# lucidrains/transfusion-pytorch

Hardware: AMD Instinct MI355X
Metric: train samples/sec, dim512 d8 seq1024 text+latent (higher is better)
Workload: dtype bf16; 1 GPU; BASELINE config 2: Transfusion dim=512 depth=8 heads=8 dim_head=64 num_text_tokens=256 dim_latent=384; per-GPU batch 64 x seq 1024 (32 x [24 text tokens + (4,384) latent] per sample); step = pack + fwd + bwd + clip(0.5) + Adam(3e-4) (one GPU: no gradient exchange); global_batch=64, seq_len=1024, parallelism=dp1

## Files before the change

include/tfx.h:

```cpp
#ifndef TFX_H
#define TFX_H
#include <stdint.h>
#ifdef __cplusplus
extern "C" {
#endif

#ifndef TFX_BF16_DEFINED
typedef uint16_t tfx_bf16;
#endif

enum { TFX_EPI_BF16 = 0, TFX_EPI_F32 = 1, TFX_EPI_SILU = 2, TFX_EPI_RESID = 3, TFX_EPI_GEGLU = 4, TFX_EPI_GEGLU_BWD = 5, TFX_EPI_QKV_NORM_ROPE = 6 };

typedef struct {
  const tfx_bf16* A; int32_t lda;
  const tfx_bf16* A2; int32_t lda2; int32_t K1;
  const tfx_bf16* B; int32_t ldb;
  int32_t M, N, K;
  int32_t epi;
  void* C; int32_t ldc;
  void* C2; int32_t ldc2;
  const float* bias;
  const tfx_bf16* R; int32_t ldr; int32_t resid_mapped;
  const int32_t* rowmap;
  const int32_t* a_rowmap;
  const tfx_bf16* aux; int32_t ldaux;
  int32_t qk_heads;
  const float* qk_gamma_q; const float* qk_gamma_k;
  const int32_t* qk_rot_pos; const float* qk_cos; const float* qk_sin;
  float qk_q_scale, qk_norm_scale;
  float* qk_plan; float qk_softcap;
  tfx_bf16* qk_cache; int32_t qk_ld_cache; const int32_t* qk_cache_pos;
  const void* prefetch; int64_t prefetch_bytes;
} tfx_gemm_nt_args;
int tfx_gemm_nt(const tfx_gemm_nt_args* a, void* stream);
int tfx_gemm_nt_plan(const tfx_gemm_nt_args* a, int32_t* kind, int32_t* grid);

int tfx_mfma_peak_probe(const void* ops, float* out, int32_t iters, int32_t blocks, void* stream);

typedef struct {
  const tfx_bf16* A; int32_t lda; int32_t a_cols;
  const tfx_bf16* B; int32_t ldb; int32_t b_cols;
  int32_t M, N, K;
  float* C; int32_t ldc;
  const int32_t* rowmap;
  int32_t k_valid;
  int32_t splits;
  int32_t accumulate;
  float alpha;
  const int32_t* a_rowmap;
  const int32_t* b_rowmap;
  float* colsum;
  int32_t k_group;
  const void* group_next;
} tfx_gemm_tn_args;
int tfx_gemm_tn(const tfx_gemm_tn_args* a, void* stream);
int tfx_gemm_tn_plan(const tfx_gemm_tn_args* a, int32_t* kind, int32_t* tiles, int32_t* splits, int32_t* grid);

typedef struct {
  const tfx_bf16 *q, *k, *v; int32_t ld_q, ld_k, ld_v;
  const tfx_bf16* gate; int32_t ld_gate;
  const int32_t* kv_end;
  const int32_t* q_start;
  tfx_bf16* out; int32_t ld_out;
  float* lse;
  int32_t b, h, n;
  float softcap;
  int32_t n_kv;
  const tfx_bf16* dout; int32_t ld_dout;
  tfx_bf16* do_eff; int32_t ld_do;
  float* delta;
  tfx_bf16* dgate; int32_t ld_dgate;
  tfx_bf16 *dq, *dk, *dv; int32_t ld_dq, ld_dk, ld_dv;
  int32_t order;
  const float* sc_plan;
  const int32_t* q_row0; const int32_t* q_cnt;
  const tfx_bf16* nr_qkv; int32_t nr_ld_qkv;
  tfx_bf16* nr_dqkv; int32_t nr_ld_dqkv;
  const float* nr_gamma_q; const float* nr_gamma_k;
  const int32_t* nr_rot_pos; const float* nr_cos; const float* nr_sin;
  float nr_q_scale, nr_norm_scale;
  float* nr_dgamma_q; float* nr_dgamma_k;
  int32_t laser;
} tfx_attn_args;
int tfx_attn_fwd(const tfx_attn_args* a, void* stream);
int tfx_attn_bwd(const tfx_attn_args* a, void* stream);

int tfx_decode_attn(const tfx_attn_args* a, void* stream);

typedef struct {
  int32_t T, H;
  const tfx_bf16* v; int32_t ld_v;
  tfx_bf16* vl; int32_t ld_vl;
  const int32_t* rowmap;
  float c;
  const tfx_bf16* dvl; int32_t ld_dvl;
  tfx_bf16* dv; int32_t ld_dv;
} tfx_laser_v_args;
int tfx_laser_v_fwd(const tfx_laser_v_args* a, void* stream);
int tfx_laser_v_bwd(const tfx_laser_v_args* a, void* stream);

typedef struct {
  int32_t T, d;
  const tfx_bf16* x; tfx_bf16* u;
  const int32_t* tok_inst;
  const float* table; int32_t ld_table;
  const float* gamma_text;
  float* mean; float* rstd;
  const tfx_bf16* du; tfx_bf16* dx;
  float* dtable;
  float* dgamma_text;
  const int32_t* seg_start; const int32_t* seg_len; int32_t n_seg;
  const tfx_bf16* dx_add;
} tfx_adaln_pre_args;
int tfx_adaln_pre_fwd(const tfx_adaln_pre_args* a, void* stream);
int tfx_adaln_pre_bwd(const tfx_adaln_pre_args* a, void* stream);

typedef struct {
  int32_t T, d;
  const tfx_bf16* x; const tfx_bf16* y; tfx_bf16* out;
  const int32_t* tok_inst;
  const float* table; int32_t ld_table;
  const float* layerscale;
  const tfx_bf16* g; tfx_bf16* dy;
  float* dtable; float* dlayerscale;
  const int32_t* seg_start; const int32_t* seg_len; int32_t n_seg;
  float* dbias;
} tfx_adaln_post_args;
int tfx_adaln_post_fwd(const tfx_adaln_post_args* a, void* stream);
int tfx_adaln_post_bwd(const tfx_adaln_post_args* a, void* stream);

typedef struct {
  int32_t T, H;
  const tfx_bf16* qkv; int32_t ld_qkv;
  tfx_bf16* qk; int32_t ld_qk;
  const float* gamma_q; const float* gamma_k;
  const int32_t* rot_pos;
// ... 54 lines not shown
typedef struct {
  int32_t T, d;
  const tfx_bf16* x; tfx_bf16* y; const float* gamma;
  const tfx_bf16* dy; tfx_bf16* dx; float* dgamma;
} tfx_rmsnorm_args;
int tfx_rmsnorm_fwd(const tfx_rmsnorm_args* a, void* stream);
int tfx_rmsnorm_bwd(const tfx_rmsnorm_args* a, void* stream);

typedef struct {
  int32_t T, d;
  const int32_t* text_ids; const int32_t* tok_inst;
  const tfx_bf16* table;
  tfx_bf16* x;
  const tfx_bf16* dx; float* dtable;
} tfx_embed_args;
int tfx_embed_fwd(const tfx_embed_args* a, void* stream);
int tfx_embed_bwd(const tfx_embed_args* a, void* stream);

typedef struct {
  int32_t R, dl;
  const float* x; const float* eps;
  const int32_t* row_inst; const float* inst_time;
  tfx_bf16* xt; int32_t ld_xt;
  float* flow;
} tfx_noise_mix_args;
int tfx_noise_mix(const tfx_noise_mix_args* a, void* stream);

typedef struct { int32_t I, half; const float* times; const float* w; tfx_bf16* out; int32_t ld; } tfx_fourier_args;
int tfx_fourier(const tfx_fourier_args* a, void* stream);

typedef struct {
  int32_t T, V; const float* logits; int32_t ld;
  const int32_t* labels;
  float grad_scale;
  tfx_bf16* dlogits; int32_t ld_d;
  float* acc;
} tfx_ce_args;
int tfx_ce_fwd_bwd(const tfx_ce_args* a, void* stream);

typedef struct {
  int32_t R, dl; const float* pred; int32_t ld_pred; const float* flow;
  float grad_scale;
  tfx_bf16* dpred; int32_t ld_d;
  float* acc;
  int32_t accumulate;
  const int32_t* row_inst; const float* inst_time; float clean_eps;
  const float* recon_w; const int32_t* recon_inst; const float* recon_time; int32_t recon_mode;
} tfx_mse_args;
int tfx_mse_fwd_bwd(const tfx_mse_args* a, void* stream);
typedef struct {
  int32_t T, d; const tfx_bf16* pred; int32_t ld_pred; const tfx_bf16* target; int32_t ld_target;
  int32_t n_pad, n_valid;
  float grad_scale;
  tfx_bf16* dpred; int32_t ld_d;
  float* acc;
} tfx_cosine_args;
int tfx_cosine_fwd_bwd(const tfx_cosine_args* a, void* stream);
int tfx_output_to_flow(float* pred, const float* x, const float* eps, const int32_t* row_inst, const float* inst_time,
                       int32_t R, int32_t dl, float clean_eps, void* stream);

int tfx_sample_tokens(const float* logits, int32_t ld, int32_t B, int32_t V, float temperature, float min_p, const float* uniforms,
                      const int32_t* active, int32_t* out_ids, void* stream);
int tfx_sample_tokens_range(const float* logits, int32_t ld, int32_t B, int32_t V, int32_t V_draw, float temperature, float min_p, const float* uniforms,
                            const int32_t* active, int32_t* out_ids, void* stream);
int tfx_ode_axpy(const float* y, const float* f_cond, const float* f_uncond, float cfg_scale, float a, float* out, int64_t n, void* stream);
int tfx_ode_stage(const float* y, const float* ym, const float* ctl, int32_t B, int32_t Lc, int32_t dmax, float* x, int32_t H, int32_t Lq, int32_t dl,
                  const int32_t* rows0, void* stream);
int tfx_ode_update(float* y, float* ym, const float* ctl, int32_t B, int32_t Lc, int32_t dmax, const float* pred, int32_t H, int32_t Lq, int32_t dl,
                   float cfg_scale, const float* sel, const int32_t* rows0, void* stream);

typedef struct { const float* src; int32_t ld_src, Rs, Cs; const int32_t* rowmap; tfx_bf16* dst; int32_t ld_dst, Rd, Cd; } tfx_cast_args;
int tfx_cast_rows(const tfx_cast_args* a, void* stream);
int tfx_cast_rows_t(const tfx_cast_args* a, void* stream);
typedef struct { const float* src; int32_t ld_src, Rs, Cs; const int32_t* rowmap; tfx_bf16* dst; int32_t ld_dst, Rd, Cd; int32_t transposed, first_block; } tfx_cast_job;
int tfx_cast_batch(const tfx_cast_job* jobs_dev, int32_t n_jobs, int32_t n_blocks, void* stream);
int tfx_gather_f32(const float* src, const int32_t* map, float* dst, int32_t n, void* stream);
int tfx_onehot_bf16(const int32_t* ids, const int32_t* tok_inst, tfx_bf16* out, int32_t T, int32_t ld, void* stream);
int tfx_scatter_rows_bf16(const tfx_bf16* src, int32_t ld_src, int32_t cols, tfx_bf16* dst, int32_t ld_dst, const int32_t* rowmap, int32_t R, void* stream);
int tfx_f32_to_bf16(const float* src, tfx_bf16* dst, int64_t n, void* stream);
int tfx_cast_block_bf16(const float* src, int32_t ld_src, tfx_bf16* dst, int32_t ld_dst, int32_t R, int32_t C, void* stream);
int tfx_silu_bwd(const tfx_bf16* dy, const tfx_bf16* pre, tfx_bf16* dx, int64_t n, void* stream);
int tfx_colsum_bf16(const tfx_bf16* src, int32_t ld, int32_t R, int32_t C, const int32_t* colmap, const int32_t* rowmap, float* out, void* stream);
int tfx_colsum_f32(const float* src, int32_t ld, int32_t R, int32_t C, float* out, void* stream);
int tfx_add_bf16(const tfx_bf16* a, const tfx_bf16* b, tfx_bf16* out, int64_t n, void* stream);
int tfx_scale_bf16_dev(tfx_bf16* x, int64_t n, const float* scale, void* stream);
int tfx_scale_bf16_copy(const tfx_bf16* src, tfx_bf16* dst, int64_t n, float scale, void* stream);

int tfx_sumsq(const float* g, int64_t n, float* sumsq, void* stream);
typedef struct {
  float* p; const float* g; float* m; float* v; int64_t n;
  float lr, beta1, beta2, eps, weight_decay, max_norm, grad_scale;
  int32_t step; const float* sumsq;
  const int64_t* skip; int32_t nskip;
} tfx_adam_args;
int tfx_adam_step(const tfx_adam_args* a, void* stream);

enum { TFX_SUMSQ_DET_PARTIALS = 1024 };
int tfx_sumsq_det(const float* g, int64_t n, float* partials, float* sumsq, void* stream);
int tfx_muon_plan(int32_t rows, int32_t cols, int32_t* flip, int32_t* m, int32_t* n, int32_t* m_pad, int32_t* n_pad, int32_t* gram_tiles,
                  int32_t* update_tiles, int32_t* prep_blocks);
int tfx_muon_step_launches(int32_t ns_steps, int32_t nmat);
typedef struct {
  int64_t off;
  int64_t s_off, t_off;
  int32_t rows, cols, ld_s, ld_t;
  int32_t blk0;
  float lr_ratio;
} tfx_muon_mat;
typedef struct {
  const tfx_muon_mat* mats; const int32_t* blk_mat; int32_t nmat, nblk;
  const float* g; float* buf; tfx_bf16* ws; float* partials;
  const float* sumsq; float max_norm, grad_scale, momentum; int32_t nesterov;
} tfx_muon_prep_args;
int tfx_muon_prep(const tfx_muon_prep_args* a, void* stream);
int tfx_muon_norm(const tfx_muon_mat* mats, int32_t nmat, const float* partials, float eps, float* inv, void* stream);
typedef struct {
  const tfx_bf16* P; const tfx_bf16* Q; const tfx_bf16* Z; tfx_bf16* C; tfx_bf16* Ct;
  const float* scale_z; const float* scale_acc;
  int32_t M, N, K, ldp, ldq, ldz, ldc, ldct;
  int32_t tile0;
  int32_t reserved;
} tfx_muon_gemm_problem;
int tfx_muon_gemm(const tfx_muon_gemm_problem* table, const int32_t* tile_prob, int32_t ntiles, float alpha, float beta, void* stream);
typedef struct {
  const tfx_muon_mat* mats; const int32_t* blk_mat; int32_t nmat, nblk;
  float* p; const tfx_bf16* ws; float lr, decay;
} tfx_muon_apply_args;
int tfx_muon_apply(const tfx_muon_apply_args* a, void* stream);
int tfx_ema_update(float* ema, const float* online, int64_t n, float decay, void* stream);

int tfx_allreduce_unique_id(void* out128);
int tfx_allreduce_init(int32_t rank, int32_t world, const void* unique_id128);
int tfx_allreduce_run(float* buf, int64_t count, void* stream);
int tfx_allreduce_destroy(void);

typedef struct { const void *p0, *p1, *p2, *p3, *p4; int64_t i0, i1, i2, i3; float f0; int32_t reserved; } tfx_raw_args;
enum { TFX_OP_GEMM_NT = 0, TFX_OP_GEMM_TN = 1, TFX_OP_ATTN_FWD = 2, TFX_OP_ATTN_BWD = 3, TFX_OP_ADALN_PRE_FWD = 4, TFX_OP_ADALN_PRE_BWD = 5,
       TFX_OP_ADALN_POST_FWD = 6, TFX_OP_ADALN_POST_BWD = 7, TFX_OP_QK_NORM_ROPE_FWD = 8, TFX_OP_QK_NORM_ROPE_BWD = 9, TFX_OP_ATTNRES_FWD = 10,
       TFX_OP_ATTNRES_BWD = 11, TFX_OP_RMSNORM_FWD = 12, TFX_OP_RMSNORM_BWD = 13, TFX_OP_EMBED_FWD = 14, TFX_OP_EMBED_BWD = 15,
       TFX_OP_NOISE_MIX = 16, TFX_OP_FOURIER = 17, TFX_OP_CE_FWD_BWD = 18, TFX_OP_MSE_FWD_BWD = 19, TFX_OP_CAST_ROWS = 20, TFX_OP_CAST_ROWS_T = 21,
       TFX_OP_ADAM_STEP = 22, TFX_OP_DECODE_ATTN = 23, TFX_OP_LASER_V_FWD = 24, TFX_OP_LASER_V_BWD = 25, TFX_OP_COSINE_FWD_BWD = 26,
       TFX_OP_OUTPUT_TO_FLOW = 32, TFX_OP_GATHER_F32 = 33, TFX_OP_ONEHOT_BF16 = 34, TFX_OP_SCATTER_ROWS_BF16 = 35, TFX_OP_F32_TO_BF16 = 36,
       TFX_OP_SILU_BWD = 37, TFX_OP_COLSUM_BF16 = 38, TFX_OP_COLSUM_F32 = 39, TFX_OP_ADD_BF16 = 40, TFX_OP_SCALE_BF16_DEV = 41, TFX_OP_CAST_BLOCK_BF16 = 42, TFX_OP_SCALE_BF16_COPY = 43, TFX_OP_ADALN_POST_PRE_FWD = 44, TFX_OP_LAYER_END_FWD = 45,
       TFX_OP_ATTNRES_PREP = 46, TFX_OP_ATTNRES_PULL_BWD = 47, TFX_OP_ATTNRES_FINISH = 52, TFX_OP_ADALN_PRE_POST_BWD = 53,
       TFX_OP_FORK = 48, TFX_OP_JOIN = 49, TFX_OP_JOIN_RECORD = 50, TFX_OP_JOIN_WAIT = 51 };
typedef struct { int32_t op; int32_t stream; const void* args; } tfx_launch;
int tfx_run_list(const tfx_launch* list, int32_t n, void* stream, int32_t* failed_at);
int tfx_graph_create(const tfx_launch* list, int32_t n, void** graph_out);
int tfx_graph_create_single(const tfx_launch* list, int32_t n, void** graph_out);
int tfx_graph_launch(void* graph, void* stream);
int tfx_graph_destroy(void* graph);
int tfx_list_fingerprint(const tfx_launch* list, int32_t n, int64_t* out);
int tfx_set_single_stream(int32_t on);

const char* tfx_version(void);

#ifdef __cplusplus
}
#endif
#endif
```

transfusion_pytorch_amd/capi.py:

```python
from __future__ import annotations

import ctypes
import os
import re

HERE = os.path.dirname(os.path.abspath(__file__))
HEADER = os.path.join(os.path.dirname(HERE), 'include', 'tfx.h')
LIB_PATH = os.environ.get('TFX_LIB') or os.path.join(HERE, 'lib', 'libtfx_hip.so')

_SCALARS = {'int32_t': ctypes.c_int32, 'int64_t': ctypes.c_int64, 'float': ctypes.c_float, 'int': ctypes.c_int}


def _strip_comments(src: str) -> str:
    src = re.sub(r'/\*.*?\*/', '', src, flags=re.S)
    return re.sub(r'//[^\n]*', '', src)


def parse_header(path: str = HEADER):
    src = _strip_comments(open(path).read())
    structs, funcs, enums = {}, {}, {}
    for body in re.findall(r'enum\s*\{(.*?)\}', src, flags=re.S):
        for item in body.split(','):
            if '=' in item:
                k, v = item.split('=')
                enums[k.strip()] = int(v.strip())
    for body, name in re.findall(r'typedef\s+struct\s*\{(.*?)\}\s*(\w+)\s*;', src, flags=re.S):
        fields = []
        for decl in body.split(';'):
            decl = decl.strip()
            if not decl:
                continue
            decl = decl.replace('const ', '')
            m = re.match(r'(\w+)\s*(.*)', decl, flags=re.S)
            base, rest = m.group(1), m.group(2)
            for d in rest.split(','):
                d = d.strip()
                is_ptr = d.startswith('*')
                fname = d.lstrip('* ').strip()
                if is_ptr:
                    fields.append((fname, ctypes.c_void_p))
                else:
                    fields.append((fname, _SCALARS[base]))
        structs[name] = fields
    for ret, name, args in re.findall(r'\b(int|const char\s*\*)\s+(tfx_\w+)\s*\(([^)]*)\)\s*;', src):
        argt = []
        for a in args.split(','):
            a = a.strip().replace('const ', '')
            if a in ('void', ''):
                continue
            if '*' in a:
                argt.append(ctypes.c_void_p)
            else:
                argt.append(_SCALARS[a.split()[0]])
        funcs[name] = (ctypes.c_char_p if 'char' in ret else ctypes.c_int, argt)
    return structs, funcs, enums


STRUCT_FIELDS, FUNCTIONS, ENUMS = parse_header()


def _make_struct(name, fields):
    return type(name, (ctypes.Structure,), {'_fields_': fields})


STRUCTS = {n: _make_struct(n, f) for n, f in STRUCT_FIELDS.items()}
_lib = None


class TfxError(RuntimeError):
    pass


def lib():
    global _lib
    if _lib is None:
        if not os.path.exists(LIB_PATH):
            raise TfxError(f'{LIB_PATH} is missing: build it with `python -m transfusion_pytorch_amd.build` '
                           '(hipcc --offload-arch=gfx950); the Transfusion hot path has no fallback')
        L = ctypes.CDLL(LIB_PATH)
        for fname, (ret, argt) in FUNCTIONS.items():
            fn = getattr(L, fname)
            fn.restype = ret
            fn.argtypes = argt
        _lib = L
    return _lib


def ptr(t):
    return None if t is None else t.data_ptr()


def make_args(struct_name: str, **kw):
    S = STRUCTS[struct_name]
    a = S()
    names = {f for f, _ in STRUCT_FIELDS[struct_name]}
    for k, v in kw.items():
        if k not in names:
            raise KeyError(f'{struct_name} has no field {k}')
        if hasattr(v, 'data_ptr'):
            v = v.data_ptr()
        setattr(a, k, v)
    return a


def check(rc: int, what: str):
    if rc != 0:
        raise TfxError(f'{what} failed with code {rc}')


def call(fn_name: str, args, stream: int):
    rc = getattr(lib(), fn_name)(ctypes.byref(args), ctypes.c_void_p(stream))
    if rc != 0:
        raise TfxError(f'{fn_name} failed with code {rc}')
```

transfusion_pytorch_amd/csrc/gemm.hip:

```cpp
#include "tfx_common.h"
#include "tfx_kernels.h"
#include <type_traits>
#include <cmath>
#include <cstring>
#include <vector>
#include <algorithm>
#include <mutex>

namespace tfx {

constexpr int BM = 128, BN = 128, BK = 64;

template <int EPI> struct Epilogue;

TFX_DEV void store_bf16x4(bf16* dst, f32x4 v) {
  bf16x4 o; o[0] = f2bf(v[0]); o[1] = f2bf(v[1]); o[2] = f2bf(v[2]); o[3] = f2bf(v[3]);
  *(bf16x4*)dst = o;
}

TFX_DEV f32x4 add_bias(const GemmNT& p, int n, f32x4 v) {
  if (p.bias) { f32x4 b = *(const f32x4*)(p.bias + n); v += b; }
  return v;
}

// ... 251 lines not shown
  for (int j = 0; j < 2; j++)
#pragma unroll
    for (int g = 0; g < 4; g++) bias[j][g] = zero4;
  if (p.bias) {
#pragma unroll
    for (int j = 0; j < 2; j++)
#pragma unroll
      for (int g = 0; g < 4; g++) bias[j][g] = *(const f32x4*)(p.bias + min(n_w + j * 32 + 8 * g + 4 * hi, p.N - 4));
  }
  const bool col_ok = n_w + ch * 8 < p.N;
  const int ncol = min(n_w + ch * 8, p.N - 8);
  bf16* sr = st + 4096;
  bf16x8 pre[4];
  auto load_r = [&](int i) {
#pragma unroll
    for (int q = 0; q < 4; q++) pre[q] = *(const bf16x8*)(p.R + (size_t)mr[i][q] * p.ldr + ncol);
  };
  load_r(0);
#pragma unroll
  for (int i = 0; i < NI; i++) {
#pragma unroll
    for (int q = 0; q < 4; q++) {
      const int row = q * 8 + (l >> 3);
      *(bf16x8*)(sr + row * 64 + ((ch ^ ((row >> 1) & 7)) << 3)) = pre[q];
    }
    if (i + 1 < NI) load_r(i + 1);
    bf16* s = st + (i & 1) * 2048;
#pragma unroll
    for (int j = 0; j < 2; j++)
#pragma unroll
      for (int g = 0; g < 4; g++) {
        const int col = j * 32 + 8 * g + 4 * hi;
        const bf16x4 rv = *(const bf16x4*)(sr + r * 64 + (((col >> 3) ^ ((r >> 1) & 7)) << 3) + (col & 7));
        f32x4 v;
#pragma unroll
        for (int e = 0; e < 4; e++) v[e] = acc[i][j][4 * g + e] + bias[j][g][e] + bf2f(rv[e]);
        stage_put4(s, r, col, v);
      }
    bf16x8 v[4];
#pragma unroll
    for (int q = 0; q < 4; q++) {
      const int row = q * 8 + (l >> 3);
      v[q] = *(const bf16x8*)(s + row * 64 + ((ch ^ ((row >> 1) & 7)) << 3));
    }
#pragma unroll
    for (int q = 0; q < 4; q++)
      if (col_ok && mo[i][q] >= 0) *(bf16x8*)((bf16*)p.C + (size_t)mo[i][q] * p.ldc + n_w + ch * 8) = v[q];
  }
}
TFX_DEV void stage_put4_32(bf16* st, int row, int col, f32x4 v) {
  bf16x4 o; o[0] = f2bf(v[0]); o[1] = f2bf(v[1]); o[2] = f2bf(v[2]); o[3] = f2bf(v[3]);
  *(bf16x4*)(st + row * 32 + (((col >> 3) ^ ((row >> 2) & 3)) << 3) + (col & 7)) = o;
}
constexpr int GTAB_N = 4096;
TFX_DEV float gelu_grid(const float* gtab, float g) {
  const float x = g * 128.f;
  const float xr = __builtin_amdgcn_fmed3f(__builtin_rintf(x), -1024.f, 1023.f);
  const float d = x - xr;
  const f32x4 c = *(const f32x4*)(gtab + 4 * ((int)xr + 1024));
  return fmaf(fmaf(c[2], d, c[1]), d, c[0]);
}
TFX_DEV GegluUVH geglu_uvh_grid(const float* gtab, float a, float g) {
  const float x = g * 128.f;
  const float xr = __builtin_amdgcn_fmed3f(__builtin_rintf(x), -1024.f, 1023.f);
  const float d = x - xr;
  const f32x4 c = *(const f32x4*)(gtab + 4 * ((int)xr + 1024));
  const float t = fmaf(c[2], d, c[1]);
  GegluUVH r; r.u = fmaf(t, d, c[0]);
  r.h = a * r.u;
  r.v = (a * 128.f) * fmaf(c[2], d, t);
  return r;
}
template <int EPI, int NI>
TFX_DEV void staged_epilogue_geglu(const GemmNT& p, f32x16 (&acc)[NI][2], int m_w, int n_w, bf16* st, const float* gtab = nullptr, bool use_tab = false) {
  const int l = threadIdx.x & 63, hi = l >> 5, r = l & 31, ch = l & 7;
  int mo[NI][4], mo2[NI][2];
#pragma unroll
  for (int i = 0; i < NI; i++) {
#pragma unroll
    for (int q = 0; q < 4; q++) { const int m = m_w + i * 32 + q * 8 + (l >> 3); mo[i][q] = m < p.M ? (p.rowmap ? p.rowmap[m] : m) : -1; }
#pragma unroll
    for (int q = 0; q < 2; q++) { const int m = m_w + i * 32 + q * 16 + (l >> 2); mo2[i][q] = (EPI == EPI_GEGLU && m < p.M) ? (p.rowmap ? p.rowmap[m] : m) : -1; }
  }
  auto flush64 = [&](const bf16* s, int i, int n_base, int Nout) {
    bf16x8 v[4];
#pragma unroll
    for (int q = 0; q < 4; q++) {
      const int row = q * 8 + (l >> 3);
      v[q] = *(const bf16x8*)(s + row * 64 + ((ch ^ ((row >> 1) & 7)) << 3));
    }
#pragma unroll
    for (int q = 0; q < 4; q++)
      if (n_base + ch * 8 < Nout && mo[i][q] >= 0) *(bf16x8*)((bf16*)p.C + (size_t)mo[i][q] * p.ldc + n_base + ch * 8) = v[q];
  };
  if constexpr (EPI == EPI_GEGLU) {
    f32x4 ba[4], bg[4];
    const f32x4 zero4 = {0.f, 0.f, 0.f, 0.f};
#pragma unroll
    for (int g = 0; g < 4; g++) { ba[g] = zero4; bg[g] = zero4; }
    if (p.bias) {
#pragma unroll
      for (int g = 0; g < 4; g++) { const int n_a = min(n_w + 8 * g + 4 * hi, p.N - 36); ba[g] = *(const f32x4*)(p.bias + n_a); bg[g] = *(const f32x4*)(p.bias + n_a + 32); }
    }
    const int c4 = l & 3;
#pragma unroll
    for (int i = 0; i < NI; i++) {
      bf16* s = st + (i & 1) * 3072;
#pragma unroll
      for (int g = 0; g < 4; g++) {
        const int nl = 8 * g + 4 * hi;
        f32x4 u, v, h;
        if (use_tab) {
#pragma unroll
          for (int e = 0; e < 4; e++) { const GegluUVH t_ = geglu_uvh_grid(gtab, acc[i][0][4 * g + e] + ba[g][e], acc[i][1][4 * g + e] + bg[g][e]); u[e] = t_.u; v[e] = t_.v; h[e] = t_.h; }
        } else {
#pragma unroll
          for (int e = 0; e < 4; e++) { const GegluUVH t_ = geglu_uvh(acc[i][0][4 * g + e] + ba[g][e], acc[i][1][4 * g + e] + bg[g][e]); u[e] = t_.u; v[e] = t_.v; h[e] = t_.h; }
        }
        stage_put4(s, r, nl, u); stage_put4(s, r, 32 + nl, v); stage_put4_32(s + 2048, r, nl, h);
      }
      flush64(s, i, n_w, p.N);
      bf16x8 hv[2];
#pragma unroll
      for (int q = 0; q < 2; q++) {
        const int row = q * 16 + (l >> 2);
        hv[q] = *(const bf16x8*)(s + 2048 + row * 32 + ((c4 ^ ((row >> 2) & 3)) << 3));
      }
      const int feat = (n_w >> 6) * 32 + c4 * 8;
#pragma unroll
      for (int q = 0; q < 2; q++)
        if (n_w < p.N && mo2[i][q] >= 0) *(bf16x8*)((bf16*)p.C2 + (size_t)mo2[i][q] * p.ldc2 + feat) = hv[q];
    }
  } else {
    bf16* sag = st + 2048;
    const int cbase = min(n_w >> 5, (p.N >> 5) - 2) * 64;
    bf16x8 pre[8];
    auto load_aux = [&](int i) {
#pragma unroll
      for (int k = 0; k < 8; k++) {
        const int q = l + 64 * k, row = q >> 4, cc = q & 15;
        const int m = min(m_w + i * 32 + row, p.M - 1);
        pre[k] = *(const bf16x8*)(p.aux + (size_t)m * p.ldaux + cbase + cc * 8);
      }
    };
    load_aux(0);
#pragma unroll
    for (int i = 0; i < NI; i++) {
#pragma unroll
      for (int k = 0; k < 8; k++) {
        const int q = l + 64 * k, row = q >> 4, cc = q & 15;
        *(bf16x8*)(sag + row * 128 + ((cc ^ (row & 15)) << 3)) = pre[k];
      }
      if (i + 1 < NI) load_aux(i + 1);
#pragma unroll
      for (int j = 0; j < 2; j++) {
#pragma unroll
        for (int g = 0; g < 4; g++) {
          const bf16x4 u4 = *(const bf16x4*)(sag + r * 128 + (((j * 8 + g) ^ (r & 15)) << 3) + 4 * hi);
          const bf16x4 v4 = *(const bf16x4*)(sag + r * 128 + (((j * 8 + 4 + g) ^ (r & 15)) << 3) + 4 * hi);
          f32x4 da, dg;
#pragma unroll
          for (int e = 0; e < 4; e++) {
            const float dh = acc[i][j][4 * g + e];
            da[e] = dh * bf2f(u4[e]);
            dg[e] = dh * bf2f(v4[e]);
          }
          stage_put4(st, r, 8 * g + 4 * hi, da); stage_put4(st, r, 32 + 8 * g + 4 * hi, dg);
        }
        if (n_w + j * 32 < p.N) flush64(st, i, ((n_w >> 5) + j) * 64, 2 * p.N);
      }
    }
  }
}
template <int NI, bool GUARD>
TFX_DEV void staged_epilogue_qknr_(const GemmNT& p, f32x16 (&acc)[NI][2], int m_w, int n_w, bf16* st) {
  const int l = threadIdx.x & 63, hi = l >> 5, r = l & 31, ch = l & 7;
  const int hd = p.qk_heads * 64;
  const int which = n_w >= hd;
  const bool col_ok = n_w + ch * 8 < p.N;
  constexpr int NS = 2 * NI;
  auto row_of = [&](int s, int k) { return m_w + (s >> 1) * 32 + (2 * (s & 1) + k) * 8 + (l >> 3); };
  f32x4 g0 = {0.f, 0.f, 0.f, 0.f}, g1 = g0;
  float rs = 0.f;
  int pos_a[2] = {0, 0}, pos_b[2] = {0, 0};
  f32x4 cs_n[2], sn_n[2];
  auto load_pos = [&](int s, int (&pos)[2]) {
#pragma unroll
    for (int k = 0; k < 2; k++) pos[k] = p.qk_rot_pos[min(row_of(s, k), p.M - 1)];
  };
  const bool to_cache = NI == 1 && p.qk_cache != nullptr && which == 1;
  int cpos[NI == 1 ? NS : 1][2];
  if constexpr (NI == 1) {
#pragma unroll
    for (int s = 0; s < NS; s++)
#pragma unroll
      for (int k = 0; k < 2; k++) { const int m = row_of(s, k); cpos[s][k] = (to_cache && m < p.M) ? p.qk_cache_pos[m] : -1; }
  }
  auto load_cs = [&](const int (&pos)[2], f32x4 (&cs)[2], f32x4 (&sn)[2]) {
#pragma unroll
    for (int k = 0; k < 2; k++) {
      cs[k] = *(const f32x4*)(p.qk_cos + (size_t)pos[k] * 32 + ch * 4);
      sn[k] = *(const f32x4*)(p.qk_sin + (size_t)pos[k] * 32 + ch * 4);
    }
  };
  {
    const float* gm = (which ? p.qk_gamma_k : p.qk_gamma_q) + ch * 8;
    g0 = *(const f32x4*)gm; g1 = *(const f32x4*)(gm + 4);
    rs = (p.qk_norm_scale > 0.f ? p.qk_norm_scale : 8.f);
    load_pos(0, pos_a);
    load_cs(pos_a, cs_n, sn_n);
    load_pos(1, pos_a);
    if (NS > 2) load_pos(2, pos_b);
    asm volatile("" ::: "memory");
  }
  bf16x8 v[4];
#pragma unroll
  for (int s = 0; s < NS; s++) {
    const int i = s >> 1, qh = s & 1;
    f32x4 cs[2] = {cs_n[0], cs_n[1]}, sn[2] = {sn_n[0], sn_n[1]};
    {
      if (s + 1 < NS) load_cs(pos_a, cs_n, sn_n);
      pos_a[0] = pos_b[0]; pos_a[1] = pos_b[1];
      if (s + 3 < NS) load_pos(s + 3, pos_b);
      asm volatile("" ::: "memory");
    }
    if (qh == 0) {
      bf16* sbuf = st + (i & 1) * 2048;
#pragma unroll
      for (int j = 0; j < 2; j++)
#pragma unroll
        for (int g = 0; g < 4; g++) {
          f32x4 a4;
#pragma unroll
          for (int e = 0; e < 4; e++) a4[e] = acc[i][j][4 * g + e];
          stage_put4(sbuf, r, j * 32 + 8 * g + 4 * hi, a4);
        }
#pragma unroll
      for (int q = 0; q < 4; q++) {
        const int row = q * 8 + (l >> 3);
        v[q] = *(const bf16x8*)(sbuf + row * 64 + ((ch ^ ((row >> 1) & 7)) << 3));
      }
#pragma unroll
      for (int q = 0; q < 4; q++) {
        const int m = m_w + i * 32 + q * 8 + (l >> 3);
        if (!GUARD || (col_ok && m < p.M)) *(bf16x8*)((bf16*)p.C + (size_t)m * p.ldc + n_w + ch * 8) = v[q];
      }
    }
    {
#pragma unroll
      for (int k = 0; k < 2; k++) {
        float gm[8];
#pragma unroll
// ... 170 lines not shown
      *(u32x4*)(As + buf * BM * BK + off) = ra[i];
      *(u32x4*)(Bs + buf * BN * BK + off) = rb[i];
    }
  };

  f32x16 acc[2][2];
#pragma unroll
  for (int i = 0; i < 2; i++)
#pragma unroll
    for (int j = 0; j < 2; j++)
#pragma unroll
      for (int r = 0; r < 16; r++) acc[i][j][r] = 0.f;

  gload(0);
  sstore(0);
  __syncthreads();

  const int arow0 = wm * 64 + (l & 31), brow0 = wn * 64 + (l & 31);
  for (int kt = 0; kt < nk; kt++) {
    const int cur = kt & 1;
    if (kt + 1 < nk) gload(kt + 1);
    const bf16* as = As + cur * BM * BK;
    const bf16* bs = Bs + cur * BN * BK;
#pragma unroll
    for (int ks = 0; ks < 4; ks++) {
      bf16x8 af[2], bfr[2];
#pragma unroll
      for (int i = 0; i < 2; i++) {
        int ar = arow0 + i * 32, br = brow0 + i * 32;
        af[i] = *(const bf16x8*)(as + ar * BK + (((ks * 2 + hi) ^ ((ar >> 1) & 7)) << 3));
        bfr[i] = *(const bf16x8*)(bs + br * BK + (((ks * 2 + hi) ^ ((br >> 1) & 7)) << 3));
      }
#pragma unroll
      for (int i = 0; i < 2; i++)
#pragma unroll
        for (int j = 0; j < 2; j++)
          acc[i][j] = __builtin_amdgcn_mfma_f32_32x32x16_bf16(bfr[j], af[i], acc[i][j], 0, 0, 0);
    }
    if (kt + 1 < nk) sstore(cur ^ 1);
    __syncthreads();
  }

#pragma unroll
  for (int i = 0; i < 2; i++) {
    const int m = m0 + wm * 64 + i * 32 + (l & 31);
    if (m >= p.M) continue;
    const int mo = p.rowmap ? p.rowmap[m] : m;
    if (mo < 0) continue;
    if constexpr (EPI == EPI_GEGLU) {
#pragma unroll
      for (int g = 0; g < 4; g++) {
        const int n_a = n0 + wn * 64 + 8 * g + 4 * hi;
        if (n_a >= p.N) continue;
        f32x4 a, gt;
#pragma unroll
        for (int e = 0; e < 4; e++) { a[e] = acc[i][0][4 * g + e]; gt[e] = acc[i][1][4 * g + e]; }
        GegluFwd::apply(p, mo, n_a, a, gt);
      }
    } else {
#pragma unroll
      for (int j = 0; j < 2; j++)
#pragma unroll
        for (int g = 0; g < 4; g++) {
          const int n = n0 + wn * 64 + j * 32 + 8 * g + 4 * hi;
          if (n >= p.N) continue;
          f32x4 v;
#pragma unroll
          for (int e = 0; e < 4; e++) v[e] = acc[i][j][4 * g + e];
          Epilogue<EPI>::apply(p, m, mo, n, v);
        }
    }
  }
}

constexpr int TN_BMK = 64;
constexpr int TN_LD = 136;

TFX_DEV int tn_out_col(const GemmTN& p, int k) {
  if (p.k_group <= 0) return k;
  const int c = k & 63;
  return c < p.k_group ? (k >> 6) * p.k_group + c : -1;
}

struct TnBlock { int tile, mbeg, mend; };
TFX_DEV TnBlock tn_block(const GemmTN& p, int ntile) {
  const int per = gridDim.x >> 3;
  const int g = (int)(blockIdx.x & 7) * per + (int)(blockIdx.x >> 3);
  TnBlock b;
  const int chunk = ((p.M + p.splits - 1) / p.splits + TN_BMK - 1) / TN_BMK * TN_BMK;
  const int split = g / ntile;
  b.tile = g - split * ntile;
  b.mbeg = split < p.splits ? min(split * chunk, p.M) : p.M;
  b.mend = min(p.M, b.mbeg + chunk);
  return b;
}

TFX_DEV TnBlock tn_block_ramp(const GemmTN& p, int ntile, int d) {
  if (d <= 0) return tn_block(p, ntile);
  const int per = gridDim.x >> 3;
  const int g = (int)(blockIdx.x & 7) * per + (int)(blockIdx.x >> 3);
  const int S = p.splits, U = p.M / TN_BMK;
  const int tri = d * S * (S - 1) / 2;
  const int c0 = (U - tri) / S, rem = U - tri - c0 * S;
  TnBlock b;
  const int split = g / ntile;
  b.tile = g - split * ntile;
  if (split >= S) { b.mbeg = b.mend = p.M; return b; }
  const int start = c0 * split + d * split * (split - 1) / 2, len = c0 + d * split + (split == S - 1 ? rem : 0);
  b.mbeg = start * TN_BMK; b.mend = (start + len) * TN_BMK;
  return b;
}

__global__ __launch_bounds__(256, 2) void gemm_tn_kernel(GemmTN p) {
  extern __shared__ __attribute__((aligned(16))) char smem_raw[];
  bf16* As = (bf16*)smem_raw;
  bf16* Bs = As + 2 * TN_BMK * TN_LD;

  const int t = threadIdx.x, l = t & 63, w = t >> 6;
  const int wn = w >> 1, wk = w & 1, hi = l >> 5;
  const int ntn = (p.N + 127) / 128, ntk = (p.K + 127) / 128;
  const int ntile = ntn * ntk;
  const TnBlock blk = tn_block(p, ntile);
  const int bid = blk.tile, mbeg = blk.mbeg, mend = blk.mend;
  const int n0 = (bid / ntk) * 128, k0 = (bid % ntk) * 128;
  if (mbeg >= mend) return;
  const int nsteps = (mend - mbeg + TN_BMK - 1) / TN_BMK;

  int srow[4], sch[4];
#pragma unroll
  for (int i = 0; i < 4; i++) { int c = t + 256 * i; srow[i] = c >> 4; sch[i] = c & 15; }
  u32x4 ra[4], rb[4];
  auto gload = [&](int st) {
    int mrow0 = mbeg + st * TN_BMK;
#pragma unroll
    for (int i = 0; i < 4; i++) {
      int m = mrow0 + srow[i];
      int ca = n0 + sch[i] * 8, cb = k0 + sch[i] * 8;
      u32x4 z = {0, 0, 0, 0};
      const bool ok = m < mend;
      const int ma = (ok && p.a_rowmap) ? p.a_rowmap[m] : m;
      const int mb = (ok && p.b_rowmap) ? p.b_rowmap[m] : m;
      ra[i] = (ok && ca < p.a_cols) ? *(const u32x4*)(p.A + (size_t)ma * p.lda + ca) : z;
      rb[i] = (ok && cb < p.b_cols) ? *(const u32x4*)(p.B + (size_t)mb * p.ldb + cb) : z;
    }
  };
  auto sstore = [&](int buf) {
#pragma unroll
    for (int i = 0; i < 4; i++) {
      int off = srow[i] * TN_LD + sch[i] * 8;
      *(u32x4*)(As + buf * TN_BMK * TN_LD + off) = ra[i];
      *(u32x4*)(Bs + buf * TN_BMK * TN_LD + off) = rb[i];
    }
  };

  f32x16 acc[2][2];
#pragma unroll
  for (int i = 0; i < 2; i++)
#pragma unroll
    for (int j = 0; j < 2; j++)
#pragma unroll
      for (int r = 0; r < 16; r++) acc[i][j][r] = 0.f;

  gload(0);
  sstore(0);
  __syncthreads();
  for (int st = 0; st < nsteps; st++) {
    const int cur = st & 1;
    if (st + 1 < nsteps) gload(st + 1);
    const bf16* as = As + cur * TN_BMK * TN_LD;
    const bf16* bs = Bs + cur * TN_BMK * TN_LD;
#pragma unroll
    for (int ks = 0; ks < 4; ks++) {
      const int r0 = ks * 16 + 8 * hi;
      bf16x8 af[2], bfr[2];
#pragma unroll
      for (int i = 0; i < 2; i++) {
        af[i] = lds_tr8(as, TN_LD, r0, r0 + 4, wn * 64 + i * 32);
        bfr[i] = lds_tr8(bs, TN_LD, r0, r0 + 4, wk * 64 + i * 32);
      }
#pragma unroll
      for (int i = 0; i < 2; i++)
#pragma unroll
        for (int j = 0; j < 2; j++)
          acc[i][j] = __builtin_amdgcn_mfma_f32_32x32x16_bf16(af[i], bfr[j], acc[i][j], 0, 0, 0);
    }
    if (st + 1 < nsteps) sstore(cur ^ 1);
    __syncthreads();
  }

#pragma unroll
  for (int i = 0; i < 2; i++)
#pragma unroll
    for (int r = 0; r < 16; r++) {
      const int n = n0 + wn * 64 + i * 32 + (r & 3) + 8 * (r >> 2) + 4 * hi;
      if (n >= p.N) continue;
      const int no = p.rowmap ? p.rowmap[n] : n;
      if (no < 0) continue;
#pragma unroll
      for (int j = 0; j < 2; j++) {
        const int k = k0 + wk * 64 + j * 32 + (l & 31);
        if (k < p.k_valid) {
          float v = acc[i][j][r] * p.alpha;
          const int ko = tn_out_col(p, k);
          if (ko >= 0) atomicAdd(p.C + (size_t)no * p.ldc + ko, v);
        }
      }
    }
}

typedef __attribute__((address_space(1))) const void gbl_void_t;
TFX_DEV void glds16(const bf16* g, bf16* lds_wave_base) {
  __builtin_amdgcn_global_load_lds((gbl_void_t*)g, (lds_void_t*)lds_wave_base, 16, 0, 0);
}

constexpr int PF_BLOCK_BYTES = 64 * 1024;
TFX_DEV bool prefetch_block(const GemmNT& p, int grid0) {
  if ((int)blockIdx.x < grid0) return false;
  const long long o0 = (long long)((int)blockIdx.x - grid0) * PF_BLOCK_BYTES + (long long)threadIdx.x * 64;
  const char* base = (const char*)p.prefetch;
  uint32_t acc = 0;
#pragma unroll
  for (int k = 0; k < PF_BLOCK_BYTES / (256 * 64); k++) {
    const long long o = o0 + (long long)k * 256 * 64;
    if (o + 4 <= (long long)p.prefetch_bytes) acc ^= *(const uint32_t*)(base + o);
  }
  asm volatile("" ::"v"(acc));
  return true;
}
static int prefetch_blocks(const GemmNT& p) {
  if (!p.prefetch || p.prefetch_bytes <= 0) return 0;
  const long long n = ((long long)p.prefetch_bytes + PF_BLOCK_BYTES - 1) / PF_BLOCK_BYTES;
  return (int)(n < 512 ? n : 512);
}

template <int EPI>
__global__ __launch_bounds__(256, 2) void gemm_nt_glds_kernel(GemmNT p, int grid0) {
  extern __shared__ __attribute__((aligned(16))) char smem_raw[];
  if (prefetch_block(p, grid0)) return;
  bf16* As = (bf16*)smem_raw;
  bf16* Bs = As + 2 * BM * BK;

  const int t = threadIdx.x, l = t & 63, hi = l >> 5;
  const int w = __builtin_amdgcn_readfirstlane(t >> 6);
  const int wm = w >> 1, wn = w & 1;
  const int ntn = (p.N + BN - 1) / BN;
  const int bid = xcd_remap(blockIdx.x, grid0);
  const int m0 = (bid / ntn) * BM, n0 = (bid % ntn) * BN;
  const int nk = p.K / BK;

  const bf16 *ga[4], *ga2[4], *gb[4];
#pragma unroll
  for (int j = 0; j < 4; j++) {
    const int row = w * 32 + j * 8 + (l >> 3);
    const int c = (l & 7) ^ ((row >> 1) & 7);
    int rm = min(m0 + row, p.M - 1);
    if (p.a_rowmap) rm = p.a_rowmap[rm];
    const int rn = min(n0 + row, p.N - 1);
    ga[j] = p.A + (size_t)rm * p.lda + c * 8;
    ga2[j] = p.A2 ? p.A2 + (size_t)rm * p.lda2 + c * 8 : nullptr;
    gb[j] = p.B + (size_t)rn * p.ldb + c * 8;
  }
  auto issue = [&](int kt, int buf) {
    const int k0 = kt * BK;
    const bool second = p.A2 && k0 >= p.K1;
#pragma unroll
    for (int j = 0; j < 4; j++) {
      glds16(second ? ga2[j] + (k0 - p.K1) : ga[j] + k0, As + buf * BM * BK + (w * 32 + j * 8) * BK);
      glds16(gb[j] + k0, Bs + buf * BN * BK + (w * 32 + j * 8) * BK);
    }
  };

  f32x16 acc[2][2];
#pragma unroll
  for (int i = 0; i < 2; i++)
#pragma unroll
    for (int j = 0; j < 2; j++)
#pragma unroll
      for (int r = 0; r < 16; r++) acc[i][j][r] = 0.f;

  issue(0, 0);
  const int arow0 = wm * 64 + (l & 31), brow0 = wn * 64 + (l & 31);
  auto ldfrag = [&](const bf16* base, int r, int ks) { return *(const bf16x8*)(base + r * BK + (((ks * 2 + hi) ^ ((r >> 1) & 7)) << 3)); };
  for (int kt = 0; kt < nk; kt++) {
    const int cur = kt & 1;
    asm volatile("s_waitcnt vmcnt(0)" ::: "memory");
    __builtin_amdgcn_s_barrier();
    if (kt + 1 < nk) issue(kt + 1, cur ^ 1);
// ... 728 lines not shown
    TN_CLK(c2)
#ifdef TFX_TN_TIMING
    ti += c2 - c1;
#endif
    const bf16* sa = S + buf * STAGE;
    const bf16* sb = sa + SA * SUBE;
    bf16x8 af[2][FA], bfr[2][FB];
#pragma unroll
    for (int ks = 0; ks < 2; ks++) {
#pragma unroll
      for (int i = 0; i < FA; i++) {
        const int c = (wn * FA + i) * 32;
        af[ks][i] = lds_tr8_swz(sa + (c >> 7) * SUBE, 16 * ks + 8 * hi, 16 * ks + 8 * hi + 4, c & 127);
      }
#pragma unroll
      for (int j = 0; j < FB; j++) {
        const int c = (wk * FB + j) * 32;
        bfr[ks][j] = lds_tr8_swz(sb + (c >> 7) * SUBE, 16 * ks + 8 * hi, 16 * ks + 8 * hi + 4, c & 127);
      }
    }
#pragma unroll
    for (int ks = 0; ks < 2; ks++)
#pragma unroll
      for (int i = 0; i < FA; i++)
#pragma unroll
        for (int j = 0; j < FB; j++) {
          if (!CHECK || (live_a[i] && live_b[j])) acc[i][j] = __builtin_amdgcn_mfma_f32_32x32x16_bf16(af[ks][i], bfr[ks][j], acc[i][j], 0, 0, 0);
          const int idx = (ks * FA + i) * FB + j;
          if (MORE && (idx & 1) && (idx >> 1) < NPW) {
            glds16_asm(gp[idx >> 1], S + nbuf * STAGE + loff[idx >> 1]);
            gp[idx >> 1] += gstep[idx >> 1];
            __builtin_amdgcn_sched_barrier(0);
          }
        }
    if (do_sum) {
#pragma unroll
      for (int ks = 0; ks < 2; ks++)
#pragma unroll
        for (int i = 0; i < (SUM ? FA : 1); i++) accs[i] = __builtin_amdgcn_mfma_f32_32x32x16_bf16(af[ks][i], ones, accs[i], 0, 0, 0);
    }
    buf = buf + 1 == NST ? 0 : buf + 1;
    nbuf = nbuf + 1 == NST ? 0 : nbuf + 1;
  };
  bool all_live = true;
#pragma unroll
  for (int i = 0; i < FA; i++) all_live = all_live && live_a[i];
#pragma unroll
  for (int j = 0; j < FB; j++) all_live = all_live && live_b[j];
  const int n_main = max(0, nst - (NST - 1));
  using yes = std::true_type; using no = std::false_type;
  if (all_live) {
    for (int st = 0; st < n_main; st++) slab(st, yes{}, no{});
    for (int st = n_main; st < nst; st++) slab(st, no{}, no{});
  } else {
    for (int st = 0; st < n_main; st++) slab(st, yes{}, yes{});
    for (int st = n_main; st < nst; st++) slab(st, no{}, yes{});
  }
  TN_STAMP(2)

  int out_row[FA][16];
#pragma unroll
  for (int i = 0; i < FA; i++)
#pragma unroll
    for (int r = 0; r < 16; r++) {
      const int n = n0 + (wn * FA + i) * 32 + (r & 3) + 8 * (r >> 2) + 4 * hi;
      out_row[i][r] = n >= p.N ? -1 : p.rowmap ? p.rowmap[n] : n;
    }
  int out_col[FB];
#pragma unroll
  for (int j = 0; j < FB; j++) {
    const int k = k0 + (wk * FB + j) * 32 + (l & 31);
    out_col[j] = k < p.k_valid ? tn_out_col(p, k) : -1;
  }
#pragma unroll
  for (int i = 0; i < FA; i++)
#pragma unroll
    for (int r = 0; r < 16; r++) {
      const int no = out_row[i][r];
      if (no < 0) continue;
      if (SUM && do_sum && (l & 31) == 0) atomicAdd(p.colsum + no, accs[SUM ? i : 0][r]);
      float* crow = p.C + (size_t)no * p.ldc;
#pragma unroll
      for (int j = 0; j < FB; j++)
        if (out_col[j] >= 0) atomicAdd(crow + out_col[j], acc[i][j][r] * p.alpha);
    }
  TN_STAMP(3)
#ifdef TFX_TN_TIMING
  asm volatile("s_waitcnt vmcnt(0)" ::: "memory");
  TN_STAMP(4)
  if (t == 0) { unsigned long long e = __builtin_readcyclecounter(); tc += stamps[2] - c2; stamps[5] = tw; stamps[6] = ti; stamps[7] = tc; (void)e; }
#endif
#undef TN_STAMP
#undef TN_CLK
}

#define OWT_OUT                                                                                                                                     \
        "=&a"(acc[0][0]), "=&a"(acc[0][1]), "=&a"(acc[0][2]), "=&a"(acc[0][3]), "=&a"(acc[1][0]), "=&a"(acc[1][1]), "=&a"(acc[1][2]), "=&a"(acc[1][3]),    \
        "=&a"(acc[2][0]), "=&a"(acc[2][1]), "=&a"(acc[2][2]), "=&a"(acc[2][3]), "=&a"(acc[3][0]), "=&a"(acc[3][1]), "=&a"(acc[3][2]), "=&a"(acc[3][3]),    \
        "+v"(raA[0]), "+v"(raA[1]), "+v"(raA[2]), "+v"(raA[3]), "+v"(raB[0]), "+v"(raB[1]), "+v"(raB[2]), "+v"(raB[3]),                                     \
        "+v"(voA), "+v"(voB), "+s"(sM), "+s"(cnt), "=&s"(so), "+s"(delta)
#define OWT_IN "s"(rsA), "s"(rsB), "s"(stA), "s"(stB), "s"(ksA), "s"(ksB)
#define OWT_CLOBBER                                                                                                                                 \
        "memory", "scc",                                                                                                                            \
        "v64", "v65", "v66", "v67", "v68", "v69", "v70", "v71", "v72", "v73", "v74", "v75", "v76", "v77", "v78", "v79",                             \
        "v80", "v81", "v82", "v83", "v84", "v85", "v86", "v87", "v88", "v89", "v90", "v91", "v92", "v93", "v94", "v95",                             \
        "v96", "v97", "v98", "v99", "v100", "v101", "v102", "v103", "v104", "v105", "v106", "v107", "v108", "v109", "v110", "v111",                 \
        "v112", "v113", "v114", "v115", "v116", "v117", "v118", "v119", "v120", "v121", "v122", "v123", "v124", "v125", "v126", "v127",             \
        "v128", "v129", "v130", "v131", "v132", "v133", "v134", "v135", "v136", "v137", "v138", "v139", "v140", "v141", "v142", "v143",             \
        "v144", "v145", "v146", "v147", "v148", "v149", "v150", "v151", "v152", "v153", "v154", "v155", "v156", "v157", "v158", "v159",             \
        "v160", "v161", "v162", "v163", "v164", "v165", "v166", "v167", "v168", "v169", "v170", "v171", "v172", "v173", "v174", "v175",             \
        "v176", "v177", "v178", "v179", "v180", "v181", "v182", "v183", "v184", "v185", "v186", "v187", "v188", "v189", "v190", "v191"
template <bool SUM>
TFX_DEV void tn_ow_body(const GemmTN& p, const TnBlock& blk) {
  extern __shared__ __attribute__((aligned(16))) char smem_raw[];
  bf16* S = (bf16*)smem_raw;
  const int t = threadIdx.x, l = t & 63, hi = l >> 5;
  const int w = __builtin_amdgcn_readfirstlane(t >> 6);
  const int wn = w >> 1, wk = w & 1;
  const int ntk = (p.K + 255) / 256;
  const int mbeg = blk.mbeg, mend = blk.mend;
  const int n0 = (blk.tile / ntk) * 256, k0 = (blk.tile % ntk) * 256;
  if (mend - mbeg < 192) return;
  const uint32_t prow = (uint32_t)((w >> 1) * 32 + (l >> 4));
  const uint32_t pchunk = (uint32_t)((l & 15) ^ (((l >> 4) & 3) << 2));
  uint32_t voA = (((uint32_t)mbeg + prow) * (uint32_t)p.lda + (uint32_t)(n0 + (w & 1) * 128) + pchunk * 8u) * 2u;
  const uint32_t ldb = (uint32_t)p.ldb, bcols = (uint32_t)p.b_cols, kb = (uint32_t)k0;
  uint32_t voB = (((uint32_t)mbeg + prow) * ldb + kb + (uint32_t)((w & 1) * 128) + pchunk * 8u) * 2u;
  const uint64_t baseA = (uint64_t)(uintptr_t)p.A, baseB = (uint64_t)(uintptr_t)p.B;
  u32x4 rsA, rsB;
  rsA[0] = __builtin_amdgcn_readfirstlane((uint32_t)baseA); rsA[1] = __builtin_amdgcn_readfirstlane((uint32_t)(baseA >> 32) & 0xffffu);
  rsA[2] = __builtin_amdgcn_readfirstlane(((uint32_t)(p.M - 1) * (uint32_t)p.lda + (uint32_t)p.a_cols) * 2u); rsA[3] = 0x00020000u;
  rsB[0] = __builtin_amdgcn_readfirstlane((uint32_t)baseB); rsB[1] = __builtin_amdgcn_readfirstlane((uint32_t)(baseB >> 32) & 0xffffu);
  rsB[2] = __builtin_amdgcn_readfirstlane(((uint32_t)(p.M - 1) * ldb + bcols) * 2u); rsB[3] = 0x00020000u;
  const uint32_t stA = __builtin_amdgcn_readfirstlane(8u * (uint32_t)p.lda), stB = __builtin_amdgcn_readfirstlane(8u * ldb);
  const uint32_t ksA = __builtin_amdgcn_readfirstlane(128u * (uint32_t)p.lda), ksB = __builtin_amdgcn_readfirstlane(128u * ldb);
  const uint32_t lds0 = (uint32_t)(size_t)(lds_void_t*)S;
  uint32_t sM = __builtin_amdgcn_readfirstlane(lds0 + (uint32_t)((w & 1) * 16384 + (w >> 1) * 8192));
  uint32_t cnt = __builtin_amdgcn_readfirstlane((uint32_t)((mend - mbeg) / 64)), so, delta = 65536u;
  uint32_t raA[4], raB[4];
  {
    const int g = l >> 4, q = l & 15;
    const int row = 8 * (g >> 1) + (q >> 2);
#pragma unroll
    for (int i = 0; i < 4; i++) {
      const int ch = (4 * i + 2 * (g & 1) + ((q & 3) >> 1)) ^ ((row & 3) << 2);
      const uint32_t off = (uint32_t)(row * 256 + ch * 16 + (q & 1) * 8);
      raA[i] = lds0 + (uint32_t)(wn * 16384) + off;
      raB[i] = lds0 + 32768u + (uint32_t)(wk * 16384) + off;
    }
  }
  f32x16 acc[4][4];
  f32x16 accs[2];
  const bool do_sum = SUM && p.colsum != nullptr && k0 == 0;
  if (do_sum) {
    u32x4 ones = {0x3f803f80u, 0x3f803f80u, 0x3f803f80u, 0x3f803f80u};
    if (wk == 0) {
      asm volatile(
#include "gemm_tn_ow_sum01.inc"
          : OWT_OUT, "=&v"(accs[0]), "=&v"(accs[1])
          : OWT_IN, "v"(ones)
          : OWT_CLOBBER);
    } else {
      asm volatile(
#include "gemm_tn_ow_sum23.inc"
          : OWT_OUT, "=&v"(accs[0]), "=&v"(accs[1])
          : OWT_IN, "v"(ones)
          : OWT_CLOBBER);
    }
  } else {
    asm volatile(
#include "gemm_tn_ow_loop.inc"
        : OWT_OUT
        : OWT_IN
        : OWT_CLOBBER);
  }

  int out_col[4];
#pragma unroll
  for (int j = 0; j < 4; j++) {
    const int k = k0 + (wk * 4 + j) * 32 + (l & 31);
    out_col[j] = k < p.k_valid ? tn_out_col(p, k) : -1;
  }
#pragma unroll
  for (int i = 0; i < 4; i++) {
    int out_row[16];
#pragma unroll
    for (int r = 0; r < 16; r++) {
      const int n = n0 + (wn * 4 + i) * 32 + (r & 3) + 8 * (r >> 2) + 4 * hi;
      out_row[r] = n >= p.N ? -1 : p.rowmap ? p.rowmap[n] : n;
    }
#pragma unroll
    for (int r = 0; r < 16; r++) {
      const int no = out_row[r];
      if (no < 0) continue;
      if (SUM && do_sum && (i >> 1) == wk && (l & 31) == 0) atomicAdd(p.colsum + no, accs[i & 1][r]);
      float* crow = p.C + (size_t)no * p.ldc;
#pragma unroll
      for (int j = 0; j < 4; j++)
        if (out_col[j] >= 0) atomicAdd(crow + out_col[j], acc[i][j][r] * p.alpha);
    }
  }
}
template <bool SUM>
__global__ __launch_bounds__(256, 1) void gemm_tn_ow_kernel(GemmTN p, int ramp) {
  const int ntn = (p.N + 255) / 256, ntk = (p.K + 255) / 256;
  tn_ow_body<SUM>(p, tn_block_ramp(p, ntn * ntk, ramp));
}
constexpr int TN_GROUP_MAX = 6;
struct TnGroup { int count; int tile_end[TN_GROUP_MAX]; GemmTN p[TN_GROUP_MAX]; };
template <bool SUM>
__global__ __launch_bounds__(256, 1) void gemm_tn_ow_group_kernel(TnGroup g, int ramp) {
  TnBlock blk = tn_block_ramp(g.p[0], g.tile_end[g.count - 1], ramp);
  int pid = 0, first = 0;
#pragma unroll
  for (int i = 0; i < TN_GROUP_MAX - 1; i++)
    if (i + 1 < g.count && blk.tile >= g.tile_end[i]) { pid = i + 1; first = g.tile_end[i]; }
  blk.tile -= first;
  tn_ow_body<SUM>(g.p[__builtin_amdgcn_readfirstlane(pid)], blk);
}
#undef OWT_OUT
#undef OWT_IN
#undef OWT_CLOBBER

static int tn_auto_splits(int M, int tiles, int kind) {
  constexpr double fill2 = 0.9, fill0 = 0.5;
  const int slots = kind == 2 ? 256 : 512;
  const double want = (kind == 2 ? fill2 : fill0) * slots;
  int s = 1;
  while (tiles * s < want && tiles * (s + 1) <= slots && s < 64 && M / (s + 1) >= 256) s++;
  return s;
}

static bool use_glds() {
  static int v = -1;
  if (v < 0) { const char* e = getenv("TFX_GEMM_GLDS"); v = (e && e[0] == '0') ? 0 : 1; }
  return v == 1;
}

enum { NT_FALLBACK = 0, NT_GLDS = 1, NT_MID = 2, NT_PP = 3, NT_SKINNY = 4, NT_DECODE = 5, NT_OW = 6, NT_OWP = 7 };

static const float* gelu_table() {
  static const float* tab[16] = {nullptr};
  static bool tried[16] = {false};
  static std::mutex mu;
  static int enabled = -1;
  std::lock_guard<std::mutex> lock(mu);
  if (enabled < 0) { const char* e = getenv("TFX_GELU_TABLE"); enabled = e ? atoi(e) : 1; }
  if (!(enabled & 1)) return nullptr;
  int dev = 0;
  if (hipGetDevice(&dev) != hipSuccess || dev < 0 || dev >= 16) return nullptr;
  if (!tried[dev]) {
    tried[dev] = true;
    std::vector<float> h(2 * GTAB_N);
    auto Phi = [](double g) { return 0.5 * erfc(-g * 0.70710678118654752440); };
    auto phi = [](double g) { return 0.39894228040143267794 * exp(-0.5 * g * g); };
    const double st = 1.0 / 128.0;
    for (int i = 0; i < 2048; i++) {
      const double g = (i - 1024) * st;
      h[4 * i] = (float)(g * Phi(g));
// ... 60 lines not shown
  if (!cus[dev]) { hipDeviceProp_t pr; cus[dev] = hipGetDeviceProperties(&pr, dev) == hipSuccess ? pr.multiProcessorCount : 256; }
  const int grid = std::min(cus[dev] / 8 * 8, (tiles + 7) / 8 * 8);
  hipLaunchKernelGGL(gemm_nt_owp_kernel<EPI>, dim3(grid), dim3(256), smem, s, p, PP_STAGGER, tiles);
}
template <int EPI> static void launch_ow(const GemmNT& p, int grid, hipStream_t s) {
  static uint32_t attr_ow = 0;
  const float* gtab = EPI == EPI_GEGLU ? gelu_table() : nullptr;
  const int smem = 2 * (BM2 * BK + BN2 * BK) * 2 + (gtab ? GTAB_N * 8 : 0);
  ensure_smem_attr((const void*)gemm_nt_ow_kernel<EPI>, 2 * (BM2 * BK + BN2 * BK) * 2 + GTAB_N * 8, attr_ow);
  hipLaunchKernelGGL(gemm_nt_ow_kernel<EPI>, dim3(grid), dim3(256), smem, s, p, PP_STAGGER, gtab);
}
template <int EPI> static int launch_nt(const GemmNT& p, hipStream_t s) {
  const NtPlan pl = nt_plan(p);
  const int smem = 2 * (BM * BK + BN * BK) * 2;
  switch (pl.kind) {
    case NT_DECODE: {
      static uint32_t attr_sd = 0;
      const int smem_sd = 4 * SD_ST * SD_SLOT * 2;
      ensure_smem_attr((const void*)gemm_nt_decode_kernel<EPI>, smem_sd, attr_sd);
      hipLaunchKernelGGL(gemm_nt_decode_kernel<EPI>, dim3(pl.grid + prefetch_blocks(p)), dim3(256), smem_sd, s, p, pl.grid);
      break;
    }
    case NT_SKINNY: {
      static uint32_t attr_sk = 0;
      const int smem_sk = SK_ST * SK_STAGE * 2;
      ensure_smem_attr((const void*)gemm_nt_skinny_kernel<EPI>, smem_sk, attr_sk);
      hipLaunchKernelGGL(gemm_nt_skinny_kernel<EPI>, dim3(pl.grid + prefetch_blocks(p)), dim3(256), smem_sk, s, p, pl.grid);
      break;
    }
    case NT_PP: launch_pp<EPI>(p, pl.grid, s); break;
    case NT_OW: if constexpr (EPI == EPI_BF16 || EPI == EPI_F32) launch_ow<EPI>(p, pl.grid, s); break;
    case NT_OWP: if constexpr (EPI == EPI_BF16) launch_owp<EPI>(p, pl.grid, s); break;
    case NT_MID: {
      static uint32_t attr_md = 0;
      const int smem_md = MD_ST * MD_STAGE * 2;
      ensure_smem_attr((const void*)gemm_nt_mid_kernel<EPI>, smem_md, attr_md);
      hipLaunchKernelGGL(gemm_nt_mid_kernel<EPI>, dim3(pl.grid + prefetch_blocks(p)), dim3(256), smem_md, s, p, pl.grid);
      break;
    }
    case NT_GLDS: hipLaunchKernelGGL(gemm_nt_glds_kernel<EPI>, dim3(pl.grid + prefetch_blocks(p)), dim3(256), smem, s, p, pl.grid); break;
    default: hipLaunchKernelGGL(gemm_nt_kernel<EPI>, dim3(pl.grid), dim3(256), smem, s, p); break;
  }
  return (int)hipGetLastError();
}

int gemm_nt_plan(const GemmNT& p, int* kind, int* grid) {
  if (p.K % BK != 0 || (p.A2 && p.K1 % BK != 0) || p.M <= 0 || p.N <= 0) return -1;
  const NtPlan pl = nt_plan(p);
  if (kind) *kind = pl.kind; if (grid) *grid = pl.grid;
  return 0;
}

static bool qknr_fusable(const GemmNT& p) {
  const int kind = nt_plan(p).kind;
  if (kind != NT_PP && kind != NT_DECODE) return false;
  if (kind == NT_PP && p.qk_cache) return false;
  const int hd = p.qk_heads * 64;
  if (p.qk_cache && (!p.qk_cache_pos || (p.qk_ld_cache & 7) || (((uintptr_t)p.qk_cache) & 15) || p.N < 3 * hd)) return false;
  return !p.rowmap && !p.a_rowmap && !p.bias && ((p.ldc | p.ldc2 | p.N) & 7) == 0 && (((uintptr_t)p.C | (uintptr_t)p.C2) & 15) == 0 && 2 * hd <= p.N && p.ldc2 >= 2 * hd;
}
static int gemm_nt_qknr(const GemmNT& p, hipStream_t s) {
  if (p.qk_heads <= 0 || !p.C2 || !p.qk_gamma_q || !p.qk_gamma_k || !p.qk_rot_pos || !p.qk_cos || !p.qk_sin) return -5;
  if (qknr_fusable(p)) {
    const NtPlan pl = nt_plan(p);
    if (pl.kind == NT_PP) { launch_pp<EPI_QKNR>(p, pl.grid, s); return (int)hipGetLastError(); }
    static uint32_t attr_sd = 0;
    const int smem_sd = 4 * SD_ST * SD_SLOT * 2;
    ensure_smem_attr((const void*)gemm_nt_decode_kernel<EPI_QKNR>, smem_sd, attr_sd);
    hipLaunchKernelGGL(gemm_nt_decode_kernel<EPI_QKNR>, dim3(pl.grid + prefetch_blocks(p)), dim3(256), smem_sd, s, p, pl.grid);
    return (int)hipGetLastError();
  }
  GemmNT q = p; q.epi = EPI_BF16; q.C2 = nullptr;
  const int rc = launch_nt<EPI_BF16>(q, s);
  if (rc) return rc;
  tfx_qk_norm_rope_args a;
  memset(&a, 0, sizeof(a));
  a.T = p.M; a.H = p.qk_heads; a.qkv = (const tfx_bf16*)p.C; a.ld_qkv = p.ldc; a.qk = (tfx_bf16*)p.C2; a.ld_qk = p.ldc2;
  a.gamma_q = p.qk_gamma_q; a.gamma_k = p.qk_gamma_k; a.rot_pos = p.qk_rot_pos; a.cos_tab = p.qk_cos; a.sin_tab = p.qk_sin;
  a.q_scale = p.qk_q_scale; a.norm_scale = p.qk_norm_scale; a.sc_plan = p.qk_plan; a.softcap = p.qk_softcap;
  a.cache = p.qk_cache; a.ld_cache = p.qk_ld_cache; a.cache_pos = p.qk_cache_pos;
  return tfx_qk_norm_rope_fwd(&a, (void*)s);
}

int gemm_nt(const GemmNT& p, hipStream_t s) {
  if (p.K % BK != 0 || (p.A2 && p.K1 % BK != 0) || p.M <= 0 || p.N <= 0) return -1;
  if ((p.lda | p.ldb) & 7) return -2;
  switch (p.epi) {
    case EPI_BF16: return launch_nt<EPI_BF16>(p, s);
    case EPI_F32: return launch_nt<EPI_F32>(p, s);
    case EPI_SILU: return launch_nt<EPI_SILU>(p, s);
    case EPI_RESID: return launch_nt<EPI_RESID>(p, s);
    case EPI_GEGLU: return (p.N % 64) ? -3 : launch_nt<EPI_GEGLU>(p, s);
    case EPI_GEGLU_BWD: return (p.N % 64) ? -3 : launch_nt<EPI_GEGLU_BWD>(p, s);
    case EPI_QKNR: return gemm_nt_qknr(p, s);
  }
  return -4;
}

template <bool SUM, int FA, int FB, int WN, int WK, int NST> static void launch_tn_wide(const GemmTN& q, int grid, hipStream_t s) {
  constexpr int smem = NST * (FA * WN + FB * WK) / 4 * MW_ROWS * 128 * 2;
  static uint32_t attr = 0;
  ensure_smem_attr((const void*)gemm_tn_wide_kernel<SUM, FA, FB, WN, WK, NST>, smem, attr);
  hipLaunchKernelGGL((gemm_tn_wide_kernel<SUM, FA, FB, WN, WK, NST>), dim3(grid), dim3(64 * WN * WK), smem, s, q);
}

struct TnPlan { int kind, tiles, splits, grid; };
static int tn_ow_mode();
static bool tn_ow_operands_ok(const GemmTN& q);
static TnPlan tn_plan(const GemmTN& q) {
#ifdef TFX_TN_TIMING
  const bool dma_ok = true;
#else
  const bool dma_ok = use_glds() && q.M % TN_BMK == 0 && !q.a_rowmap && !q.b_rowmap && q.a_cols >= 8 && q.b_cols >= 8;
#endif
  const int t44 = ((q.N + 255) / 256) * ((q.K + 255) / 256), t22 = ((q.N + 127) / 128) * ((q.K + 127) / 128);
  TnPlan pl;
  pl.kind = !dma_ok ? -1 : (t44 >= 8 ? 2 : 0);
  pl.tiles = pl.kind == 2 ? t44 : t22;
  pl.splits = q.splits == 0 ? tn_auto_splits(q.M, pl.tiles, pl.kind) : q.splits;
  pl.grid = (pl.tiles * pl.splits + 7) / 8 * 8;
  if (tn_ow_mode() && pl.kind == 2 && tn_ow_operands_ok(q)) {
    const int chunk = ((q.M + pl.splits - 1) / pl.splits + TN_BMK - 1) / TN_BMK * TN_BMK;
    const int last = q.M % chunk == 0 ? chunk : q.M % chunk;
    if (chunk >= 192 && last >= 192) pl.kind = 3;
  }
  return pl;
}
struct TnGroupPlan { bool ok; int count, tiles, splits, grid; TnGroup g; };
static int tn_ow_mode() {
  static int tnow = -1;
  if (tnow < 0) { const char* e = getenv("TFX_TN_OW"); tnow = e ? atoi(e) : 1; }
  return tnow;
}
static bool tn_ow_operands_ok(const GemmTN& q) {
  const long long lim = 1ll << 32;
  const bool b_ok = q.b_cols >= q.K;
  return use_glds() && q.M % 64 == 0 && !q.a_rowmap && !q.b_rowmap && (((uintptr_t)q.A | (uintptr_t)q.B) & 15) == 0 && ((q.lda | q.ldb | q.a_cols | q.b_cols) & 7) == 0 &&
         (long long)(q.M + 64) * q.lda * 2 < lim && (long long)(q.M + 64) * q.ldb * 2 < lim && q.a_cols >= q.N && b_ok && q.N > 0 && q.K > 0;
}
static TnGroupPlan tn_group_plan(const GemmTN& head) {
  TnGroupPlan gp; memset(&gp, 0, sizeof(gp));
  static int grp = -1;
  if (grp < 0) { const char* e = getenv("TFX_TN_GROUP"); grp = e ? atoi(e) : 1; }
  const GemmTN* q = &head;
  int n = 0, tiles = 0;
  bool ok = grp != 0 && tn_ow_mode() != 0;
  while (q && n < TN_GROUP_MAX) {
    ok = ok && q->M == head.M && tn_ow_operands_ok(*q);
    tiles += ((q->N + 255) / 256) * ((q->K + 255) / 256);
    gp.g.p[n] = *q; gp.g.p[n].group_next = nullptr; gp.g.tile_end[n] = tiles;
    n++;
    q = (const GemmTN*)q->group_next;
  }
  ok = ok && q == nullptr && n >= 2;
  gp.count = n; gp.tiles = tiles; gp.g.count = n;
  if (!ok) return gp;
  gp.splits = head.splits == 0 ? tn_auto_splits(head.M, tiles, 2) : head.splits;
  const int chunk = ((head.M + gp.splits - 1) / gp.splits + TN_BMK - 1) / TN_BMK * TN_BMK;
  const int last = head.M % chunk == 0 ? chunk : head.M % chunk;
  if (chunk < 192 || last < 192) return gp;
  gp.grid = (tiles * gp.splits + 7) / 8 * 8;
  if (head.splits == 0 && tiles * gp.splits < 0.8 * 256) return gp;
  for (int i = 0; i < n; i++) gp.g.p[i].splits = gp.splits;
  gp.ok = true;
  return gp;
}
static int tn_ramp(int M, int tiles, int splits) {
  constexpr int ramp_min = 8;
  int ramp = 0;
  if (splits >= ramp_min && M % TN_BMK == 0) {
    const int S = splits, U = M / TN_BMK;
    ramp = (int)(0.148 * tiles + 0.5);
    while (ramp > 0 && (U - ramp * S * (S - 1) / 2) / S < 8) ramp--;
  }
  return ramp;
}

int gemm_tn_plan(const GemmTN& p, int* kind, int* tiles, int* splits, int* grid) {
  if (p.M <= 0 || p.N <= 0 || p.K <= 0 || p.splits < 0) return -1;
  if (p.group_next) {
    const TnGroupPlan gp = tn_group_plan(p);
    if (gp.ok) { if (kind) *kind = 3; if (tiles) *tiles = gp.tiles; if (splits) *splits = gp.splits; if (grid) *grid = gp.grid; return 0; }
  }
  const TnPlan pl = tn_plan(p);
  if (kind) *kind = pl.kind; if (tiles) *tiles = pl.tiles; if (splits) *splits = pl.splits; if (grid) *grid = pl.grid;
  return 0;
}

int gemm_tn(const GemmTN& p, hipStream_t s) {
  if (p.M <= 0 || p.N <= 0 || p.K <= 0 || p.splits < 0) return -1;
  if ((p.lda | p.ldb | p.a_cols | p.b_cols) & 7) return -2;
  if (p.group_next) {
    const TnGroupPlan gp = tn_group_plan(p);
    if (gp.ok) {
      bool sum = false;
      for (int i = 0; i < gp.count; i++) sum = sum || gp.g.p[i].colsum != nullptr;
      const int ramp = tn_ramp(p.M, gp.tiles, gp.splits);
      static uint32_t attr_g0 = 0, attr_g1 = 0;
      if (sum) { ensure_smem_attr((const void*)gemm_tn_ow_group_kernel<true>, 131072, attr_g1); hipLaunchKernelGGL(gemm_tn_ow_group_kernel<true>, dim3(gp.grid), dim3(256), 131072, s, gp.g, ramp); }
      else { ensure_smem_attr((const void*)gemm_tn_ow_group_kernel<false>, 131072, attr_g0); hipLaunchKernelGGL(gemm_tn_ow_group_kernel<false>, dim3(gp.grid), dim3(256), 131072, s, gp.g, ramp); }
      return (int)hipGetLastError();
    }
    int guard = 0;
    for (const GemmTN* q = &p; q; q = (const GemmTN*)q->group_next) {
      if (++guard > 64) return -7;
      GemmTN one = *q; one.group_next = nullptr;
      const int rc = gemm_tn(one, s);
      if (rc) return rc;
    }
    return 0;
  }
  static uint32_t attr_set = 0;
  const int smem = 2 * 2 * TN_BMK * TN_LD * 2;
  ensure_smem_attr((const void*)gemm_tn_kernel, smem, attr_set);
  GemmTN q = p;
  const TnPlan pl = tn_plan(q);
  q.splits = pl.splits;
  const int kind = pl.kind, grid = pl.grid;
  if (kind == 3) {
    static uint32_t attr_tnow = 0;
    const int ramp = tn_ramp(q.M, pl.tiles, q.splits);
    if (q.colsum) {
      static uint32_t attr_tnows = 0;
      ensure_smem_attr((const void*)gemm_tn_ow_kernel<true>, 131072, attr_tnows);
      hipLaunchKernelGGL(gemm_tn_ow_kernel<true>, dim3(grid), dim3(256), 131072, s, q, ramp);
    } else {
      ensure_smem_attr((const void*)gemm_tn_ow_kernel<false>, 131072, attr_tnow);
      hipLaunchKernelGGL(gemm_tn_ow_kernel<false>, dim3(grid), dim3(256), 131072, s, q, ramp);
    }
  } else if (kind == 2) {
    if (q.colsum) launch_tn_wide<true, 2, 4, 4, 2, 4>(q, grid, s);
    else launch_tn_wide<false, 2, 4, 4, 2, 4>(q, grid, s);
  } else if (kind == 0) {
    if (q.colsum) launch_tn_wide<true, 2, 2, 2, 2, 4>(q, grid, s);
    else launch_tn_wide<false, 2, 2, 2, 2, 4>(q, grid, s);
  }
  else {
    hipLaunchKernelGGL(gemm_tn_kernel, dim3(grid), dim3(256), smem, s, q);
    if (q.colsum)
      return tfx_colsum_bf16((const tfx_bf16*)q.A, q.lda, q.M, q.N, q.rowmap, q.a_rowmap, q.colsum, (void*)s);
  }
  return (int)hipGetLastError();
}

}
```

transfusion_pytorch_amd/csrc/runner.hip:

```cpp
#include <atomic>
#include <hip/hip_runtime.h>
#include <cstdlib>
#include <cstdint>
#include "../../include/tfx.h"

namespace {

inline int run_one(const tfx_launch& l, void* s) {
  const void* a = l.args;
  const tfx_raw_args* r = static_cast<const tfx_raw_args*>(a);
  switch (l.op) {
    case TFX_OP_GEMM_NT:          return tfx_gemm_nt(static_cast<const tfx_gemm_nt_args*>(a), s);
    case TFX_OP_GEMM_TN:          return tfx_gemm_tn(static_cast<const tfx_gemm_tn_args*>(a), s);
    case TFX_OP_ATTN_FWD:         return tfx_attn_fwd(static_cast<const tfx_attn_args*>(a), s);
    case TFX_OP_ATTN_BWD:         return tfx_attn_bwd(static_cast<const tfx_attn_args*>(a), s);
    case TFX_OP_ADALN_PRE_FWD:    return tfx_adaln_pre_fwd(static_cast<const tfx_adaln_pre_args*>(a), s);
    case TFX_OP_ADALN_PRE_BWD:    return tfx_adaln_pre_bwd(static_cast<const tfx_adaln_pre_args*>(a), s);
    case TFX_OP_ADALN_POST_FWD:   return tfx_adaln_post_fwd(static_cast<const tfx_adaln_post_args*>(a), s);
    case TFX_OP_ADALN_POST_BWD:   return tfx_adaln_post_bwd(static_cast<const tfx_adaln_post_args*>(a), s);
    case TFX_OP_QK_NORM_ROPE_FWD: return tfx_qk_norm_rope_fwd(static_cast<const tfx_qk_norm_rope_args*>(a), s);
    case TFX_OP_QK_NORM_ROPE_BWD: return tfx_qk_norm_rope_bwd(static_cast<const tfx_qk_norm_rope_args*>(a), s);
    case TFX_OP_ATTNRES_FWD:      return tfx_attnres_fwd(static_cast<const tfx_attnres_args*>(a), s);
    case TFX_OP_ATTNRES_BWD:      return tfx_attnres_bwd(static_cast<const tfx_attnres_args*>(a), s);
    case TFX_OP_RMSNORM_FWD:      return tfx_rmsnorm_fwd(static_cast<const tfx_rmsnorm_args*>(a), s);
    case TFX_OP_RMSNORM_BWD:      return tfx_rmsnorm_bwd(static_cast<const tfx_rmsnorm_args*>(a), s);
    case TFX_OP_EMBED_FWD:        return tfx_embed_fwd(static_cast<const tfx_embed_args*>(a), s);
    case TFX_OP_EMBED_BWD:        return tfx_embed_bwd(static_cast<const tfx_embed_args*>(a), s);
    case TFX_OP_NOISE_MIX:        return tfx_noise_mix(static_cast<const tfx_noise_mix_args*>(a), s);
    case TFX_OP_FOURIER:          return tfx_fourier(static_cast<const tfx_fourier_args*>(a), s);
    case TFX_OP_CE_FWD_BWD:       return tfx_ce_fwd_bwd(static_cast<const tfx_ce_args*>(a), s);
    case TFX_OP_MSE_FWD_BWD:      return tfx_mse_fwd_bwd(static_cast<const tfx_mse_args*>(a), s);
    case TFX_OP_CAST_ROWS:        return tfx_cast_rows(static_cast<const tfx_cast_args*>(a), s);
    case TFX_OP_CAST_ROWS_T:      return tfx_cast_rows_t(static_cast<const tfx_cast_args*>(a), s);
    case TFX_OP_ADAM_STEP:        return tfx_adam_step(static_cast<const tfx_adam_args*>(a), s);
    case TFX_OP_DECODE_ATTN:      return tfx_decode_attn(static_cast<const tfx_attn_args*>(a), s);
    case TFX_OP_LASER_V_FWD:      return tfx_laser_v_fwd(static_cast<const tfx_laser_v_args*>(a), s);
    case TFX_OP_LASER_V_BWD:      return tfx_laser_v_bwd(static_cast<const tfx_laser_v_args*>(a), s);
    case TFX_OP_COSINE_FWD_BWD:   return tfx_cosine_fwd_bwd(static_cast<const tfx_cosine_args*>(a), s);
    case TFX_OP_OUTPUT_TO_FLOW:
      return tfx_output_to_flow((float*)r->p0, (const float*)r->p1, (const float*)r->p2, (const int32_t*)r->p3, (const float*)r->p4,
                                (int32_t)r->i0, (int32_t)r->i1, r->f0, s);
    case TFX_OP_GATHER_F32:
      return tfx_gather_f32((const float*)r->p0, (const int32_t*)r->p1, (float*)r->p2, (int32_t)r->i0, s);
    case TFX_OP_ONEHOT_BF16:
      return tfx_onehot_bf16((const int32_t*)r->p0, (const int32_t*)r->p1, (tfx_bf16*)r->p2, (int32_t)r->i0, (int32_t)r->i1, s);
    case TFX_OP_SCATTER_ROWS_BF16:
      return tfx_scatter_rows_bf16((const tfx_bf16*)r->p0, (int32_t)r->i0, (int32_t)r->i1, (tfx_bf16*)r->p1, (int32_t)r->i2,
                                   (const int32_t*)r->p2, (int32_t)r->i3, s);
    case TFX_OP_F32_TO_BF16:
      return tfx_f32_to_bf16((const float*)r->p0, (tfx_bf16*)r->p1, r->i0, s);
    case TFX_OP_SILU_BWD:
      return tfx_silu_bwd((const tfx_bf16*)r->p0, (const tfx_bf16*)r->p1, (tfx_bf16*)r->p2, r->i0, s);
    case TFX_OP_COLSUM_BF16:
      return tfx_colsum_bf16((const tfx_bf16*)r->p0, (int32_t)r->i0, (int32_t)r->i1, (int32_t)r->i2, (const int32_t*)r->p1,
                             (const int32_t*)r->p2, (float*)r->p3, s);
    case TFX_OP_COLSUM_F32:
      return tfx_colsum_f32((const float*)r->p0, (int32_t)r->i0, (int32_t)r->i1, (int32_t)r->i2, (float*)r->p1, s);
    case TFX_OP_ADD_BF16:
      return tfx_add_bf16((const tfx_bf16*)r->p0, (const tfx_bf16*)r->p1, (tfx_bf16*)r->p2, r->i0, s);
    case TFX_OP_ADALN_POST_PRE_FWD:
      return tfx_adaln_post_pre_fwd((const tfx_adaln_post_args*)r->p0, (const tfx_adaln_pre_args*)r->p1, s);
    case TFX_OP_LAYER_END_FWD:
      return tfx_layer_end_fwd((const tfx_adaln_post_args*)r->p0, (const tfx_attnres_args*)r->p1, (const tfx_adaln_pre_args*)r->p2, s);
    case TFX_OP_ATTNRES_PREP:
      return tfx_attnres_prep((const tfx_attnres_src*)r->p0, (int32_t)r->i0, (int32_t)r->i1, s);
    case TFX_OP_ATTNRES_FINISH:
      return tfx_attnres_finish((const tfx_attnres_src*)r->p0, (int32_t)r->i0, (int32_t)r->i1, s);
    case TFX_OP_ATTNRES_PULL_BWD:
      return tfx_attnres_pull_bwd((const tfx_attnres_pull_args*)r->p0, (const tfx_adaln_post_args*)r->p1, s);
    case TFX_OP_ADALN_PRE_POST_BWD:
      return tfx_adaln_pre_post_bwd((const tfx_adaln_pre_args*)r->p0, (const tfx_adaln_post_args*)r->p1, s);
    case TFX_OP_CAST_BLOCK_BF16:
      return tfx_cast_block_bf16((const float*)r->p0, (int32_t)r->i0, (tfx_bf16*)r->p1, (int32_t)r->i1, (int32_t)r->i2, (int32_t)r->i3, s);
    case TFX_OP_SCALE_BF16_COPY:
      return tfx_scale_bf16_copy((const tfx_bf16*)r->p0, (tfx_bf16*)r->p1, r->i0, r->f0, s);
    case TFX_OP_SCALE_BF16_DEV:
      return tfx_scale_bf16_dev((tfx_bf16*)r->p0, r->i0, (const float*)r->p1, s);
    default: return -100;
  }
}

struct SideStream {
  hipStream_t stream = nullptr;
  hipEvent_t fork_ev[64] = {}, join_ev[64] = {};
  int ensure() {
    if (stream) return 0;
    int lo = 0, hi = 0;
    (void)hipDeviceGetStreamPriorityRange(&lo, &hi);
    if (hipStreamCreateWithPriority(&stream, hipStreamNonBlocking, lo) != hipSuccess) return -110;
    for (int i = 0; i < 64; ++i)
      if (hipEventCreateWithFlags(&fork_ev[i], hipEventDisableTiming) != hipSuccess ||
          hipEventCreateWithFlags(&join_ev[i], hipEventDisableTiming) != hipSuccess) return -111;
    return 0;
  }
};
constexpr int kMaxDevices = 16;
SideStream g_sides[kMaxDevices];
std::atomic<bool> g_single_stream{false};
thread_local int t_force_single = 0;
inline bool single_stream() { return t_force_single > 0 || g_single_stream.load(std::memory_order_relaxed); }
inline SideStream* side_of_current_device() {
  int dev = 0;
  if (hipGetDevice(&dev) != hipSuccess || dev < 0 || dev >= kMaxDevices) return nullptr;
  return &g_sides[dev];
}

}

extern "C" int tfx_run_list(const tfx_launch* list, int32_t n, void* stream, int32_t* failed_at) {
  if (n < 0 || (n > 0 && !list)) return -1;
  hipStream_t main_s = (hipStream_t)stream;
  SideStream* sp = nullptr;
  auto side = [&](int& rc) -> SideStream* {
    if (!sp && !(sp = side_of_current_device())) { rc = -112; return nullptr; }
    rc = sp->ensure();
    return rc == 0 ? sp : nullptr;
  };
  for (int32_t i = 0; i < n; ++i) {
    const tfx_launch& l = list[i];
    int rc = 0;
    if (!l.args) rc = -2;
    else if (l.op >= TFX_OP_FORK && l.op <= TFX_OP_JOIN_WAIT) {
      if (l.stream < 0 || l.stream >= 64) rc = -3;
      else if (single_stream()) rc = 0;
      else if (SideStream* gs = side(rc)) {
        SideStream& g_side = *gs;
        if (l.op == TFX_OP_FORK) {
          rc = (int)hipEventRecord(g_side.fork_ev[l.stream], main_s);
          if (rc == 0) rc = (int)hipStreamWaitEvent(g_side.stream, g_side.fork_ev[l.stream], 0);
        } else {
          if (l.op != TFX_OP_JOIN_WAIT) rc = (int)hipEventRecord(g_side.join_ev[l.stream], g_side.stream);
          if (rc == 0 && l.op != TFX_OP_JOIN_RECORD) rc = (int)hipStreamWaitEvent(main_s, g_side.join_ev[l.stream], 0);
        }
      }
    } else if (l.stream == 1 && !single_stream()) {
      if (SideStream* gs = side(rc)) rc = run_one(l, (void*)gs->stream);
    } else if (l.stream == 1) {
      rc = run_one(l, stream);
    } else if (l.stream == 0) {
      rc = run_one(l, stream);
    } else rc = -3;
    if (rc != 0) { if (failed_at) *failed_at = i; return rc; }
  }
  return 0;
}

namespace {
hipStream_t g_capture_streams[kMaxDevices] = {};
}
extern "C" int tfx_graph_create(const tfx_launch* list, int32_t n, void** graph_out) {
  if (!graph_out || n <= 0 || !list) return -1;
  *graph_out = nullptr;
  int dev = 0;
  if (hipGetDevice(&dev) != hipSuccess || dev < 0 || dev >= kMaxDevices) return -112;
  hipStream_t& g_capture_stream = g_capture_streams[dev];
  if (!g_capture_stream && hipStreamCreateWithFlags(&g_capture_stream, hipStreamNonBlocking) != hipSuccess) return -120;
// ... 97 lines not shown
```

transfusion_pytorch_amd/csrc/tokenwise.hip:

```cpp
#include "tfx_kernels.h"
#include <map>
#include <mutex>
#include <utility>
#include <cstdlib>

namespace tfx {

constexpr int WAVES = 4;
constexpr int MAXB = 1024;

template <int NC> struct Row {
  float v[NC][8];
};

template <int NC> TFX_DEV void load_row(Row<NC>& r, const bf16* p, int d, int lane) {
#pragma unroll
  for (int i = 0; i < NC; i++) {
    int c = lane + 64 * i;
    if (c * 8 < d) {
      bf16x8 x = *(const bf16x8*)(p + c * 8);
#pragma unroll
      for (int e = 0; e < 8; e++) r.v[i][e] = bf2f(x[e]);
    } else {
#pragma unroll
// ... 1762 lines not shown
  if (i >= n) return;
  float x = bf2f(pre[i]), s = sigmoidf_(x);
  dx[i] = f2bf(bf2f(dy[i]) * s * (1.f + x * (1.f - s)));
}
__global__ void add_bf16_k(const bf16* a, const bf16* b, bf16* o, long long n) {
  long long i = ((long long)blockIdx.x * blockDim.x + threadIdx.x) * 8;
  if (i + 7 < n) {
    bf16x8 x = *(const bf16x8*)(a + i), y = *(const bf16x8*)(b + i), r;
#pragma unroll
    for (int e = 0; e < 8; e++) r[e] = f2bf(bf2f(x[e]) + bf2f(y[e]));
    *(bf16x8*)(o + i) = r;
  } else for (; i < n; i++) o[i] = f2bf(bf2f(a[i]) + bf2f(b[i]));
}

__global__ void scale_bf16_dev_k(bf16* x, long long n, const float* scale) {
  const float sc = *scale;
  if (sc == 1.f) return;
  long long i = ((long long)blockIdx.x * blockDim.x + threadIdx.x) * 8;
  if (i + 7 < n) {
    bf16x8 v = *(const bf16x8*)(x + i);
#pragma unroll
    for (int e = 0; e < 8; e++) v[e] = f2bf(bf2f(v[e]) * sc);
    *(bf16x8*)(x + i) = v;
  } else for (; i < n; i++) x[i] = f2bf(bf2f(x[i]) * sc);
}

template <typename T> __global__ __launch_bounds__(256) void colsum_k(const T* src, int ld, int R, int C, const int* colmap, const int* rowmap, float* out, int rows_per_block) {
  __shared__ float s[4][64];
  const int cx = threadIdx.x & 63, ry = threadIdx.x >> 6;
  const int c = blockIdx.x * 64 + cx;
  const int rbeg = blockIdx.y * rows_per_block, rend = min(R, rbeg + rows_per_block);
  float a = 0.f;
  if (c < C) for (int r = rbeg + ry; r < rend; r += 4) a += (float)src[(size_t)(rowmap ? rowmap[r] : r) * ld + c];
  s[ry][cx] = a;
  __syncthreads();
  if (ry == 0 && c < C) {
    float v = s[0][cx] + s[1][cx] + s[2][cx] + s[3][cx];
    int co = colmap ? colmap[c] : c;
    if (co >= 0 && v != 0.f) atomicAdd(out + co, v);
  }
}

__global__ __launch_bounds__(512) void colsum8_k(const bf16* src, int ld, int R, int C, const int* colmap, const int* rowmap, float* out, int rows_per_block) {
  __shared__ float s[8][64][9];
  const int cx = threadIdx.x & 63, ry = threadIdx.x >> 6;
  const int c0 = (blockIdx.x * 64 + cx) * 8;
  const int rbeg = blockIdx.y * rows_per_block, rend = min(R, rbeg + rows_per_block);
  float a[8];
#pragma unroll
  for (int e = 0; e < 8; e++) a[e] = 0.f;
  if (c0 < C) {
    int r = rbeg + ry;
    for (; r + 56 < rend; r += 64) {
      bf16x8 v[8];
#pragma unroll
      for (int u = 0; u < 8; u++) v[u] = *(const bf16x8*)(src + (size_t)(rowmap ? rowmap[r + 8 * u] : r + 8 * u) * ld + c0);
#pragma unroll
      for (int u = 0; u < 8; u++)
#pragma unroll
        for (int e = 0; e < 8; e++) a[e] += bf2f(v[u][e]);
    }
    for (; r < rend; r += 8) {
      bf16x8 v = *(const bf16x8*)(src + (size_t)(rowmap ? rowmap[r] : r) * ld + c0);
#pragma unroll
      for (int e = 0; e < 8; e++) a[e] += bf2f(v[e]);
    }
  }
#pragma unroll
  for (int e = 0; e < 8; e++) s[ry][cx][e] = a[e];
  __syncthreads();
  {
    const int cc = threadIdx.x >> 3, e = threadIdx.x & 7;
    const int col = (blockIdx.x * 64 + cc) * 8 + e;
    if (col < C) {
      float v = 0.f;
#pragma unroll
      for (int y = 0; y < 8; y++) v += s[y][cc][e];
      const int co = colmap ? colmap[col] : col;
      if (co >= 0 && v != 0.f) atomicAdd(out + co, v);
    }
  }
}

__global__ __launch_bounds__(256) void sumsq_k(const float* g, long long n, float* out) {
  __shared__ float sacc[WAVES];
  float s = 0.f;
  for (long long i = ((long long)blockIdx.x * blockDim.x + threadIdx.x) * 4; i < n; i += (long long)gridDim.x * blockDim.x * 4) {
    if (i + 3 < n) { f32x4 v = *(const f32x4*)(g + i); s += v[0] * v[0] + v[1] * v[1] + v[2] * v[2] + v[3] * v[3]; }
    else for (long long j = i; j < n; j++) s += g[j] * g[j];
  }
  s = wave_sum(s);
  if ((threadIdx.x & 63) == 0) sacc[threadIdx.x >> 6] = s;
  __syncthreads();
  if (threadIdx.x == 0) { float a = 0.f; for (int i = 0; i < WAVES; i++) a += sacc[i]; atomicAdd(out, a); }
}

__global__ __launch_bounds__(256) void adam_k(tfx_adam_args p, float step_size, float inv_sqrt_bc2) {
  const long long i = ((long long)blockIdx.x * blockDim.x + threadIdx.x) * 4;
  if (i >= p.n) return;
  if (p.nskip > 0) {
    int lo = 0, hi = p.nskip;
    while (lo < hi) { const int mid = (lo + hi) >> 1; if (p.skip[2 * mid + 1] > i) hi = mid; else lo = mid + 1; }
    if (lo < p.nskip && p.skip[2 * lo] <= i) return;
  }
  float coef = p.grad_scale;
  if (p.max_norm > 0.f) {
    float norm = sqrtf(p.sumsq[0]) * p.grad_scale;
    coef *= fminf(1.f, p.max_norm / (norm + 1e-6f));
  }
  if (i + 4 <= p.n) {
    const f32x4 g4 = *(const f32x4*)(p.g + i), w4 = *(const f32x4*)(p.p + i);
    f32x4 m4 = *(const f32x4*)(p.m + i), v4 = *(const f32x4*)(p.v + i), o4;
#pragma unroll
    for (int e = 0; e < 4; e++) {
      float g = g4[e] * coef;
      if (p.weight_decay != 0.f) g += p.weight_decay * w4[e];
      m4[e] = p.beta1 * m4[e] + (1.f - p.beta1) * g;
      v4[e] = p.beta2 * v4[e] + (1.f - p.beta2) * g * g;
      o4[e] = w4[e] - step_size * m4[e] / (sqrtf(v4[e]) * inv_sqrt_bc2 + p.eps);
    }
    *(f32x4*)(p.m + i) = m4; *(f32x4*)(p.v + i) = v4; *(f32x4*)(p.p + i) = o4;
  } else {
    for (long long j = i; j < p.n; j++) {
      float g = p.g[j] * coef;
      const float w = p.p[j];
      if (p.weight_decay != 0.f) g += p.weight_decay * w;
      const float m = p.beta1 * p.m[j] + (1.f - p.beta1) * g;
      const float v = p.beta2 * p.v[j] + (1.f - p.beta2) * g * g;
      p.m[j] = m; p.v[j] = v;
      p.p[j] = w - step_size * m / (sqrtf(v) * inv_sqrt_bc2 + p.eps);
    }
  }
}

__global__ __launch_bounds__(256) void output_to_flow_k(float* pred, const float* x, const float* eps, const int* row_inst, const float* inst_time,
                                                        int R, int dl, float clean_eps) {
  const int i = blockIdx.x * blockDim.x + threadIdx.x;
  if (i >= R * dl) return;
  const int r = i / dl;
  const float t = inst_time[row_inst[r]];
  const float noised = eps ? x[i] * t + eps[i] * (1.f - t) : x[i];
  pred[i] = (pred[i] - noised) / fmaxf(1.f - t, clean_eps);
}

__global__ __launch_bounds__(256) void ema_k(float* ema, const float* online, long long n, float decay) {
  const long long i = ((long long)blockIdx.x * blockDim.x + threadIdx.x) * 4;
  if (i + 4 <= n) {
    f32x4 e = *(const f32x4*)(ema + i); const f32x4 o = *(const f32x4*)(online + i);
#pragma unroll
    for (int k = 0; k < 4; k++) e[k] = o[k] + decay * (e[k] - o[k]);
    *(f32x4*)(ema + i) = e;
  } else {
    for (long long j = i; j < n; j++) ema[j] = online[j] + decay * (ema[j] - online[j]);
  }
}

TFX_DEV float laser_factor(float x, float c, float ic, float* th_out) {
  const float th = tanhf(x * ic);
  *th_out = th;
  return expf(c * th);
}
__global__ __launch_bounds__(256) void laser_v_fwd_k(tfx_laser_v_args p, unsigned nch) {
  const unsigned gid = blockIdx.x * blockDim.x + threadIdx.x;
  const unsigned cpr = (unsigned)p.H * 8;
  if (gid >= nch) return;
  const unsigned t = gid / cpr, c8 = gid - t * cpr;
// ... 175 lines not shown
int tfx_qk_norm_rope_bwd(const tfx_qk_norm_rope_args* a, void* s) {
  long long nthreads = (long long)a->T * 2 * a->H * 8;
  if (nthreads >= (1ll << 31)) return -3;
  long long g = (nthreads + 1023) / 1024;
  const long long cap = 256;
  if (g > cap) g = cap;
  hipLaunchKernelGGL(qk_norm_rope_bwd_k, dim3((unsigned)g), dim3(1024), 0, ST(s), *a); RET();
}
int tfx_noise_mix(const tfx_noise_mix_args* a, void* s) {
  long long n = (long long)a->R * a->ld_xt; if (n == 0) return 0;
  hipLaunchKernelGGL(noise_mix_k, dim3((unsigned)((n + 255) / 256)), dim3(256), 0, ST(s), *a); RET();
}
int tfx_fourier(const tfx_fourier_args* a, void* s) { if (a->I == 0) return 0; hipLaunchKernelGGL(fourier_k, dim3(a->I), dim3(256), 0, ST(s), *a); RET(); }
int tfx_ce_fwd_bwd(const tfx_ce_args* a, void* s) {
  int g = grid_tokens(a->T); if (g > 1024) g = 1024;
  hipLaunchKernelGGL(ce_k, dim3(g), dim3(256), 0, ST(s), *a); RET();
}
int tfx_mse_fwd_bwd(const tfx_mse_args* a, void* s) {
  long long n = (long long)a->R * a->ld_d; if (n == 0) return 0;
  long long g = (n + 255) / 256; if (g > 2048) g = 2048;
  hipLaunchKernelGGL(mse_k, dim3((unsigned)g), dim3(256), 0, ST(s), *a); RET();
}
int tfx_cosine_fwd_bwd(const tfx_cosine_args* a, void* s) {
  if (!a || a->T < 0 || a->d <= 0 || a->d > 2048 || (a->d % 64) || (a->ld_pred % 8) || (a->ld_target % 8) || (a->ld_d % 8) || a->ld_pred < a->d || a->ld_target < a->d || a->ld_d < a->d) return -1;
  if (!a->pred || !a->target || !a->dpred || !a->acc || a->n_pad < 0 || a->n_valid < 0) return -2;
  if (a->T == 0) return 0;
  DISPATCH_NC(a->d, hipLaunchKernelGGL(cosine_k<NC>, dim3(grid_capped(a->T)), dim3(256), 0, ST(s), *a)); RET();
}
int tfx_cast_rows(const tfx_cast_args* a, void* s) {
  long long n = (long long)a->Rd * a->ld_dst; if (n == 0) return 0;
  hipLaunchKernelGGL(cast_rows_k, dim3((unsigned)((n + 255) / 256)), dim3(256), 0, ST(s), *a); RET();
}
int tfx_cast_rows_t(const tfx_cast_args* a, void* s) {
  hipLaunchKernelGGL(cast_rows_t_k, dim3((a->ld_dst + 31) / 32, (a->Rd + 31) / 32), dim3(256), 0, ST(s), *a); RET();
}
int tfx_cast_batch(const tfx_cast_job* jobs_dev, int32_t n_jobs, int32_t n_blocks, void* s) {
  if (n_jobs <= 0 || n_blocks <= 0) return 0;
  hipLaunchKernelGGL(cast_batch_k, dim3(n_blocks), dim3(256), 0, ST(s), jobs_dev, n_jobs); RET();
}
int tfx_onehot_bf16(const int32_t* ids, const int32_t* tok_inst, tfx_bf16* out, int32_t T, int32_t ld, void* s) {
  if (T == 0) return 0; if (ld % 8) return -1;
  long long n = (long long)T * ld / 8;
  hipLaunchKernelGGL(onehot_k, dim3((unsigned)((n + 255) / 256)), dim3(256), 0, ST(s), ids, tok_inst, out, T, ld); RET();
}
int tfx_scatter_rows_bf16(const tfx_bf16* src, int32_t ld_src, int32_t cols, tfx_bf16* dst, int32_t ld_dst, const int32_t* rowmap, int32_t R, void* s) {
  if (R == 0) return 0; if (cols % 8 || ld_src % 8 || ld_dst % 8) return -1;
  long long n = (long long)R * (cols / 8);
  hipLaunchKernelGGL(scatter_rows_k, dim3((unsigned)((n + 255) / 256)), dim3(256), 0, ST(s), src, ld_src, cols, dst, ld_dst, rowmap, R); RET();
}
int tfx_gather_f32(const float* src, const int32_t* map, float* dst, int32_t n, void* s) {
  if (n == 0) return 0; hipLaunchKernelGGL(gather_f32_k, dim3((n + 255) / 256), dim3(256), 0, ST(s), src, map, dst, n); RET();
}
int tfx_f32_to_bf16(const float* src, tfx_bf16* dst, int64_t n, void* s) {
  if (n == 0) return 0; hipLaunchKernelGGL(f32_to_bf16_k, dim3((unsigned)((n / 4 + 256) / 256)), dim3(256), 0, ST(s), src, dst, (long long)n); RET();
}
int tfx_silu_bwd(const tfx_bf16* dy, const tfx_bf16* pre, tfx_bf16* dx, int64_t n, void* s) {
  if (n == 0) return 0; hipLaunchKernelGGL(silu_bwd_k, dim3((unsigned)((n + 255) / 256)), dim3(256), 0, ST(s), dy, pre, dx, (long long)n); RET();
}
int tfx_add_bf16(const tfx_bf16* a, const tfx_bf16* b, tfx_bf16* o, int64_t n, void* s) {
  if (n == 0) return 0; hipLaunchKernelGGL(add_bf16_k, dim3((unsigned)((n / 8 + 256) / 256)), dim3(256), 0, ST(s), a, b, o, (long long)n); RET();
}
int tfx_scale_bf16_dev(tfx_bf16* x, int64_t n, const float* scale, void* s) {
  if (n == 0) return 0;
  if (!x || !scale) return -1;
  hipLaunchKernelGGL(scale_bf16_dev_k, dim3((unsigned)((n / 8 + 256) / 256)), dim3(256), 0, ST(s), x, (long long)n, scale); RET();
}
static inline int colsum_rows_per_block(int R) { int rpb = (R + 63) / 64; return rpb < 4 ? 4 : rpb; }
int tfx_colsum_bf16(const tfx_bf16* src, int32_t ld, int32_t R, int32_t C, const int32_t* colmap, const int32_t* rowmap, float* out, void* s) {
  if (R == 0 || C == 0) return 0;
  if (C % 8 == 0 && ld % 8 == 0) {
    const int gx = (C + 511) / 512;
    int gy = 768 / gx; if (gy < 1) gy = 1;
    int rpb8 = (R + gy - 1) / gy; if (rpb8 < 64) rpb8 = 64;
    hipLaunchKernelGGL(colsum8_k, dim3(gx, (R + rpb8 - 1) / rpb8), dim3(512), 0, ST(s), src, ld, R, C, colmap, rowmap, out, rpb8); RET();
  }
  int rpb = colsum_rows_per_block(R);
  hipLaunchKernelGGL(colsum_k<bf16>, dim3((C + 63) / 64, (R + rpb - 1) / rpb), dim3(256), 0, ST(s), src, ld, R, C, colmap, rowmap, out, rpb); RET();
}
int tfx_colsum_f32(const float* src, int32_t ld, int32_t R, int32_t C, float* out, void* s) {
  if (R == 0 || C == 0) return 0;
  int rpb = colsum_rows_per_block(R);
  hipLaunchKernelGGL(colsum_k<float>, dim3((C + 63) / 64, (R + rpb - 1) / rpb), dim3(256), 0, ST(s), src, ld, R, C, (const int*)nullptr, (const int*)nullptr, out, rpb); RET();
}
int tfx_sumsq(const float* g, int64_t n, float* out, void* s) {
  if (n == 0) return 0;
  long long blocks = (n / 4 + 255) / 256; if (blocks > 2048) blocks = 2048; if (blocks < 1) blocks = 1;
  hipLaunchKernelGGL(sumsq_k, dim3((unsigned)blocks), dim3(256), 0, ST(s), g, (long long)n, out); RET();
}
int tfx_adam_step(const tfx_adam_args* a, void* s) {
  if (a->n == 0) return 0;
  if (((uintptr_t)a->p | (uintptr_t)a->g | (uintptr_t)a->m | (uintptr_t)a->v) & 15) return -1;
  if (a->nskip < 0 || (a->nskip > 0 && !a->skip)) return -1;
  const double bc1 = 1.0 - pow((double)a->beta1, (double)a->step), bc2 = 1.0 - pow((double)a->beta2, (double)a->step);
  const long long nthr = (a->n + 3) / 4;
  hipLaunchKernelGGL(adam_k, dim3((unsigned)((nthr + 255) / 256)), dim3(256), 0, ST(s), *a, (float)(a->lr / bc1), (float)(1.0 / sqrt(bc2))); RET();
}
int tfx_output_to_flow(float* pred, const float* x, const float* eps, const int32_t* row_inst, const float* inst_time,
                       int32_t R, int32_t dl, float clean_eps, void* s) {
  if (R <= 0 || dl <= 0) return 0;
  if ((long long)R * dl >= (1ll << 31)) return -1;
  hipLaunchKernelGGL(output_to_flow_k, dim3((unsigned)(((long long)R * dl + 255) / 256)), dim3(256), 0, ST(s), pred, x, eps, row_inst, inst_time, R, dl, clean_eps); RET();
}
int tfx_ema_update(float* ema, const float* online, int64_t n, float decay, void* s) {
  if (n <= 0) return 0;
  if (((uintptr_t)ema | (uintptr_t)online) & 15) return -1;
  hipLaunchKernelGGL(ema_k, dim3((unsigned)(((n + 3) / 4 + 255) / 256)), dim3(256), 0, ST(s), ema, online, (long long)n, decay); RET();
}
int tfx_gemm_nt(const tfx_gemm_nt_args* a, void* s) { return gemm_nt(*a, ST(s)); }
int tfx_gemm_tn(const tfx_gemm_tn_args* a, void* s) { return gemm_tn(*a, ST(s)); }
int tfx_gemm_nt_plan(const tfx_gemm_nt_args* a, int32_t* kind, int32_t* grid) { return gemm_nt_plan(*a, kind, grid); }
int tfx_gemm_tn_plan(const tfx_gemm_tn_args* a, int32_t* kind, int32_t* tiles, int32_t* splits, int32_t* grid) { return gemm_tn_plan(*a, kind, tiles, splits, grid); }
int tfx_attn_fwd(const tfx_attn_args* a, void* s) { return attn_fwd(*a, ST(s)); }
int tfx_attn_bwd(const tfx_attn_args* a, void* s) { return attn_bwd(*a, ST(s)); }
int tfx_mfma_peak_probe(const void* ops, float* out, int32_t iters, int32_t blocks, void* s) {
  if (!ops || !out || iters <= 0 || blocks <= 0) return -1;
  hipLaunchKernelGGL(mfma_peak_k, dim3(blocks), dim3(256), 0, ST(s), (const bf16x8*)ops, out, iters); RET();
}
int tfx_laser_v_fwd(const tfx_laser_v_args* a, void* s) {
  if (!a || a->T < 0 || a->H <= 0 || !(a->c > 0.f)) return -1;
  if (a->T == 0) return 0;
  if (!a->v || !a->vl || ((a->ld_v | a->ld_vl) & 7) || a->ld_v < a->H * 64 || a->ld_vl < a->H * 64 || (((uintptr_t)a->v | (uintptr_t)a->vl) & 15)) return -2;
  const long long nch = (long long)a->T * a->H * 8;
  if (nch >= (1ll << 31)) return -4;
  hipLaunchKernelGGL(laser_v_fwd_k, dim3((unsigned)((nch + 255) / 256)), dim3(256), 0, ST(s), *a, (unsigned)nch); RET();
}
int tfx_laser_v_bwd(const tfx_laser_v_args* a, void* s) {
  if (!a || a->T < 0 || a->H <= 0 || !(a->c > 0.f)) return -1;
  if (a->T == 0) return 0;
  if (!a->v || !a->dvl || !a->dv || ((a->ld_v | a->ld_dvl | a->ld_dv) & 7) || a->ld_v < a->H * 64 || a->ld_dvl < a->H * 64 || a->ld_dv < a->H * 64 ||
      (((uintptr_t)a->v | (uintptr_t)a->dvl | (uintptr_t)a->dv) & 15)) return -2;
  const long long nch = (long long)a->T * a->H * 8;
  if (nch >= (1ll << 31)) return -4;
  hipLaunchKernelGGL(laser_v_bwd_k, dim3((unsigned)((nch + 255) / 256)), dim3(256), 0, ST(s), *a, (unsigned)nch); RET();
}
const char* tfx_version(void) { return "tfx-hip gfx950 r4-laser-muon-selfflow"; }

}
```

transfusion_pytorch_amd/engine.py:

```python
from __future__ import annotations

import ctypes
import os
import weakref

import torch

from . import capi
from .params import ModelDims, ParamStore, pad_to

BF16 = torch.bfloat16
E = capi.ENUMS


def _p(t, *idx):
    for i in idx:
        t = t[i]
    return t.data_ptr()


def skip_sources(md: ModelDims):
    stack, src = [], {}
    for i in range(md.depth):
        layer = i + 1
        if layer <= md.depth // 2:
            stack.append(i)
        elif md.has_skip(i):
            src[i] = stack.pop()
    assert not stack
    return src




_LAUNCH = capi.STRUCTS['tfx_launch']
_RAW = capi.STRUCTS['tfx_raw_args']


def raw_args(fn_name: str, values):
    argt = capi.FUNCTIONS[fn_name][1][:-1]
    assert len(argt) == len(values), f'{fn_name}: {len(values)} arguments for {len(argt)} parameters'
    r = _RAW()
    np_, ni, nf = 0, 0, 0
    for ty, v in zip(argt, values):
        if ty is ctypes.c_void_p:
            setattr(r, f'p{np_}', v); np_ += 1
        elif ty is ctypes.c_float:
            assert nf == 0
            r.f0 = v; nf += 1
        else:
            setattr(r, f'i{ni}', v); ni += 1
    return r


class Side(tuple):
    """a launch that runs on the library's side stream (include/tfx.h `tfx_launch.stream` = 1): the weight-gradient GEMMs, next to
    the data-gradient chain on the caller's stream.  Unpacks like any other (entry point, args) item."""


_AUTO_AFTER = 2
TRAIN_GRAPH = os.environ.get('TFX_TRAIN_GRAPH', '0') == '1'
_SYNC_OPS = {'tfx_fork': 'TFX_OP_FORK', 'tfx_join': 'TFX_OP_JOIN', 'tfx_join_record': 'TFX_OP_JOIN_RECORD', 'tfx_join_wait': 'TFX_OP_JOIN_WAIT'}
_DUMMY = ctypes.c_int32(0)


class LaunchList(list):
    _image = None
    _graphs = None
    meta = None

    def graph(self, lo: int, hi: int):
        if self._graphs is None:
            self._graphs = {}
        g = self._graphs.get((lo, hi))
        if g is None:
            arr = self.native()
            out = ctypes.c_void_p()
            rc = capi.lib().tfx_graph_create(ctypes.byref(arr, lo * ctypes.sizeof(_LAUNCH)), hi - lo, ctypes.byref(out))
            if rc != 0 or not out.value:
                raise capi.TfxError(f'tfx_graph_create failed with code {rc}')
            g = self._graphs[(lo, hi)] = out.value
        return g

    def invalidate_graphs(self):
        for g in (self._graphs or {}).values():
            capi.lib().tfx_graph_destroy(ctypes.c_void_p(g))
        self._graphs = None
        for st in (self._auto or {}).values():
            if st[1]:
                capi.lib().tfx_graph_destroy(ctypes.c_void_p(st[1]))
        self._auto = None

    _auto = None

    def replay_auto(self, lo: int, hi: int, sp) -> bool:
        lib = capi.lib()
        arr = self.native()
        fp = ctypes.c_int64()
        rc = lib.tfx_list_fingerprint(ctypes.byref(arr, lo * ctypes.sizeof(_LAUNCH)), hi - lo, ctypes.byref(fp))
        if rc != 0:
            return False
        if self._auto is None:
            self._auto = {}
        st = self._auto.get((lo, hi))
        if st is None or st[0] != fp.value:
            if st is not None and st[1]:
                lib.tfx_graph_destroy(ctypes.c_void_p(st[1]))
            self._auto[(lo, hi)] = [fp.value, None, 0]
            return False
        st[2] += 1
        if st[1] is None:
            if st[2] < _AUTO_AFTER:
                return False
            out = ctypes.c_void_p()
            rc = lib.tfx_graph_create_single(ctypes.byref(arr, lo * ctypes.sizeof(_LAUNCH)), hi - lo, ctypes.byref(out))
# ... 530 lines not shown
                    self._nt(C, algo_k=dl, A=lt['ndpred'], lda=dlp, B=S[f'outp_t{t}'], ldb=dlp, M=r, N=d, K=dlp, epi=E['TFX_EPI_BF16'], C=lt['dpx'], ldc=d)
                    self._tn(C, r, d, dl, A=lt['dpx'], lda=d, a_cols=d, B=lt['xt'], ldb=dlp, b_cols=dlp, C=gp(f'latent_to_model_projs.{t}.weight'), ldc=dl)
                    self._raw(C, lib.tfx_colsum_bf16, lt['dpx'].data_ptr(), d, r, d, None, None, gp(f'latent_to_model_projs.{t}.bias'))
        self._nt(L, algo_k=md.vocab, A=self.dlogits, lda=md.vp, B=S['logits_t'], ldb=md.vp, M=T, N=d, K=md.vp, epi=E['TFX_EPI_BF16'], C=self.dembed, ldc=d)
        self._tn(L, T, md.vocab, d, A=self.dlogits, lda=md.vp, a_cols=md.vp, B=self.embed, ldb=d, b_cols=d, C=gp('to_text_logits.weight'), ldc=d)
        for t, r in self.R.items():
            dl = md.dim_latents[t]; dlp = pad_to(dl, 64); lt = self.lat[t]
            if t in self.ext:
                self._nt(L, A=lt['gemb'], lda=d, B=S['eye'], ldb=d, M=r, N=d, K=d, epi=E['TFX_EPI_RESID'], C=self.dembed, ldc=d,
                         R=self.dembed, ldr=d, resid_mapped=1, rowmap=self.row_tok[t])
                continue
            self._nt(L, algo_k=dl, A=lt['dpred'], lda=dlp, B=S[f'outp_t{t}'], ldb=dlp, M=r, N=d, K=dlp, epi=E['TFX_EPI_RESID'], C=self.dembed, ldc=d,
                     R=self.dembed, ldr=d, resid_mapped=1, rowmap=self.row_tok[t])
            self._tn(L, r, dl, d, A=lt['dpred'], lda=dlp, a_cols=dlp, B=self.embed, ldb=d, b_cols=d, b_rowmap=self.row_gat[t],
                     C=gp(f'model_to_latent_projs.{t}.weight'), ldc=d)
        self.tap_final = len(L)
        self._k(L, 'tfx_rmsnorm_bwd', 'tfx_rmsnorm_args', T=T, d=d, x=self.xres[D], gamma=pp('transformer.norm.gamma'), dy=self.dembed,
                dx=self.gfin, dgamma=gp('transformer.norm.gamma'))
        self._hbm(L, 3)
        src = skip_sources(md)
        pushed = set(src.values())
        g = self.gfin
        side = self.side
        def sync(op, slot):
            if side:
                L.append((op, slot))
        pull = self.pull
        if pull:
            self.dsum = torch.empty(D, T, device=ps.device, dtype=torch.float32)
            self.wtab = torch.empty(2, D, d, device=ps.device, dtype=torch.float32)
            self.nbytes += self.dsum.numel() * 4 + self.wtab.numel() * 4
            SRC = capi.STRUCTS['tfx_attnres_src']
            recs = (SRC * D)()
            for j in range(D):
                pj = f'transformer.layers.{j}.3'
                gj = self.gfin if j == D - 1 else (self.gx[j + 1] if md.has_skip(j + 1) else self.dH[j + 2])
                for k, v in dict(g=gj, save=self.arsave[j], dsum=self.dsum[j], w=self.wtab[0, j], dw=self.wtab[1, j], gamma=pp(f'{pj}.norm_keys.gamma'),
                                 pq=pp(f'{pj}.pseudo_queries'), dgamma=gp(f'{pj}.norm_keys.gamma'), dpq=gp(f'{pj}.pseudo_queries'), L=j + 2).items():
                    setattr(recs[j], k, v.data_ptr() if hasattr(v, 'data_ptr') else v)
            raw = torch.frombuffer(bytearray(ctypes.string_at(ctypes.addressof(recs), ctypes.sizeof(recs))), dtype=torch.uint8)
            self._src_tab = raw.to(ps.device)
            self._src_size = ctypes.sizeof(SRC)
            self._raw(L, lib.tfx_attnres_prep, self._src_tab.data_ptr(), D, d)
        self._pull_args = {}
        def pull_launch(l, out_own, add, dh, post):
            j0 = max(l - 1, 0)
            ns = D - j0
            export = ns > 8 or d > 512
            if export and not hasattr(self, 'k1buf'):
                self.k1buf = torch.zeros(T, 32, device=ps.device, dtype=BF16); self.nbytes += self.k1buf.numel() * 2
            a = capi.make_args('tfx_attnres_pull_args', T=T, d=d, l=l, n_src=ns, h=self.hid[l], src=self._src_tab.data_ptr() + j0 * self._src_size,
                               out_own=out_own, out_err=self.arerr[l - 1] if out_own is not None else None, add=add, dh=dh,
                               seg_start=self.seg_start, seg_len=self.seg_len, n_seg=0, k1=self.k1buf if export else None, ld_k1=32)
            self._seg_args.append(a)
            self._pull_args[l] = a
            self._keep = getattr(self, '_keep', []) + [a, post]
            self._raw(L, lib.tfx_attnres_pull_bwd, ctypes.addressof(a), ctypes.addressof(post) if post is not None else None)
            self._hbm(L, ns + 6 if post is not None else ns + 4, 12 * ns * T)
            if export:
                self._tn(L, T, ns, d, A=self.k1buf, lda=32, a_cols=32, B=self.hid[l], ldb=d, b_cols=d, C=self.wtab[1, j0], ldc=d)
        for i in range(D - 1, -1, -1):
            p = f'transformer.layers.{i}'
            x_in = self.xres[i]
            x_a = self.xa[i] if md.has_skip(i) else x_in
            (ta, dta), (tf, dtf) = self._tab(i, 0), self._tab(i, 1)
            par = i % len(self.dag_p)
            dy_f, dy_a, dag, dqkvg = self.dy_f[par], self.dy_a[par], self.dag_p[par], self.dqkvg_p[par]
            if i + 2 <= D - 1:
                sync('tfx_join_wait', i + 2)
            G = self.dH[i + 1]
            a_postf = capi.make_args('tfx_adaln_post_args', T=T, d=d, y=self.yf[i], tok_inst=self.tok_inst, table=tf, ld_table=nt3,
                                     layerscale=pp(f'{p}.2.layerscale'), g=G, dy=dy_f, dtable=dtf, dlayerscale=gp(f'{p}.2.layerscale'),
                                     seg_start=self.seg_start, seg_len=self.seg_len, n_seg=0, dbias=gp(f'{p}.2.fn.net.3.bias'))
            self._seg_args.append(a_postf)
            if pull:
                pull_launch(i + 1, self.xres[i + 1], None, G, a_postf)
            else:
                g2 = self.dskip[i + 1] if (i + 1) in pushed else None
                self._k(L, 'tfx_attnres_bwd', 'tfx_attnres_args', T=T, d=d, L=i + 2, hiddens=self.hid, stride_h=T * d,
                        gamma=pp(f'{p}.3.norm_keys.gamma'), pq=pp(f'{p}.3.pseudo_queries'), g=g, g2=capi.ptr(g2), dhiddens=self.dH, stride_dh=T * d,
                        first=1 if i == D - 1 else 0, dgamma=gp(f'{p}.3.norm_keys.gamma'), dpq=gp(f'{p}.3.pseudo_queries'))
                L.append(('tfx_adaln_post_bwd', a_postf))
            self._nt(L, algo_n=di, A=dy_f, lda=d, B=S[f'ff2_t{i}'], ldb=d, M=T, N=dip, K=d, epi=E['TFX_EPI_GEGLU_BWD'], C=dag, ldc=2 * dip,
                     aux=self.ag[i], ldaux=2 * dip)
            sync('tfx_fork', 2 * i)
            ff_grp = [(d, di, dict(A=dy_f, lda=d, a_cols=d, B=self.hm[i], ldb=dip, b_cols=dip, C=gp(f'{p}.2.fn.net.3.weight'), ldc=di)),
                      (2 * dip, d, dict(algo_n=2 * di, A=dag, lda=2 * dip, a_cols=2 * dip, B=self.uf[i], ldb=d, b_cols=d, rowmap=gmap,
                                        C=gp(f'{p}.2.fn.net.0.weight'), ldc=d, colsum=gp(f'{p}.2.fn.net.0.bias')))]
            self._tn_group(L, T, ff_grp, side=side)
            self._nt(L, algo_k=2 * di, A=dag, lda=2 * dip, B=S[f'ff1_t{i}'], ldb=2 * dip, M=T, N=d, K=2 * dip, epi=E['TFX_EPI_BF16'], C=self.du, ldc=d)
            a_pref = capi.make_args('tfx_adaln_pre_args', T=T, d=d, x=self.xb[i], tok_inst=self.tok_inst, table=tf, ld_table=nt3,
                                    gamma_text=pp(f'{p}.2.layernorm_gamma'), mean=_p(self.stats, 2, i), rstd=_p(self.stats, 3, i), du=self.du, dx=G,
                                    dtable=dtf, dgamma_text=gp(f'{p}.2.layernorm_gamma'), seg_start=self.seg_start, seg_len=self.seg_len, n_seg=0)
            a_posta = capi.make_args('tfx_adaln_post_args', T=T, d=d, y=self.ya[i], tok_inst=self.tok_inst, table=ta, ld_table=nt3,
                                     layerscale=pp(f'{p}.1.layerscale'), g=G, dy=dy_a, dtable=dta, dlayerscale=gp(f'{p}.1.layerscale'),
                                     seg_start=self.seg_start, seg_len=self.seg_len, n_seg=0)
            self._seg_args += [a_pref, a_posta]
            self._keep = getattr(self, '_keep', []) + [a_pref, a_posta]
            self._raw(L, lib.tfx_adaln_pre_post_bwd, ctypes.addressof(a_pref), ctypes.addressof(a_posta))
            self._hbm(L, 6)
            self._nt(L, algo_n=md.hd, A=dy_a, lda=d, B=S[f'out_t{i}'], ldb=d, M=T, N=hd, K=d, epi=E['TFX_EPI_BF16'], C=self.dog, ldc=hd)
            gam = (lambda nm: S[f'g{nm}{i}']) if md.dim_head != 64 else (lambda nm: pp(f'{p}.1.fn.{nm}_norm.gamma'))
            if os.environ.get('TFX_ATTN_QKNR', '1') != '0':
                self._k(L, 'tfx_attn_bwd', 'tfx_attn_args', **self._attn_kw(i, bwd=True), nr_qkv=self.qkvg[i], nr_ld_qkv=ldq, nr_dqkv=dqkvg, nr_ld_dqkv=ldq,
                        nr_gamma_q=gam('q'), nr_gamma_k=gam('k'), nr_rot_pos=self.rot_pos, nr_cos=0, nr_sin=0, nr_q_scale=md.dim_head ** -0.5,
                        nr_norm_scale=md.dim_head ** 0.5, nr_dgamma_q=gp(f'{p}.1.fn.q_norm.gamma'), nr_dgamma_k=gp(f'{p}.1.fn.k_norm.gamma'))
                self._rope_attn_args = getattr(self, '_rope_attn_args', []) + [L[-1][1]]
            else:
                self._k(L, 'tfx_attn_bwd', 'tfx_attn_args', **self._attn_kw(i, bwd=True))
                self._k(L, 'tfx_qk_norm_rope_bwd', 'tfx_qk_norm_rope_args', T=T, H=H, qkv=self.qkvg[i], ld_qkv=ldq, gamma_q=gam('q'),
                        gamma_k=gam('k'), rot_pos=self.rot_pos, cos_tab=0, sin_tab=0, q_scale=md.dim_head ** -0.5, norm_scale=md.dim_head ** 0.5,
                        dqk=self.dqk, ld_dqk=2 * hd, dqkv=dqkvg, ld_dqkv=ldq, dgamma_q=gp(f'{p}.1.fn.q_norm.gamma'), dgamma_k=gp(f'{p}.1.fn.k_norm.gamma'))
                self._rope_args = getattr(self, '_rope_args', []) + [L[-1][1]]
                L.meta = L.meta or {}
                L.meta[len(L) - 1] = ('hbm', 3 * 2 * T * hd * 2)
            if md.laser:
                dv = dqkvg.data_ptr() + 2 * 2 * hd
                self._k(L, 'tfx_laser_v_bwd', 'tfx_laser_v_args', T=T, H=H, v=_p(self.qkvg, i) + 2 * 2 * hd, ld_v=ldq, c=md.laser,
                        dvl=dv, ld_dvl=ldq, dv=dv, ld_dv=ldq)
                L.meta = L.meta or {}
                L.meta[len(L) - 1] = ('hbm', 3 * T * hd * 2)
            self._nt(L, algo_k=md.nq, A=dqkvg, lda=ldq, B=S[f'qkvg_t{i}'], ldb=ldq, M=T, N=d, K=ldq, epi=E['TFX_EPI_BF16'], C=self.du, ldc=d)
            self._k(L, 'tfx_adaln_pre_bwd', 'tfx_adaln_pre_args', T=T, d=d, x=x_a, tok_inst=self.tok_inst, table=ta, ld_table=nt3,
                    gamma_text=pp(f'{p}.1.layernorm_gamma'), mean=_p(self.stats, 0, i), rstd=_p(self.stats, 1, i), du=self.du, dx=G,
                    dtable=dta, dgamma_text=gp(f'{p}.1.layernorm_gamma'), seg_start=self.seg_start, seg_len=self.seg_len, n_seg=0,
                    dx_add=self.dskip[i] if (pull and i in pushed) else None)
            self._hbm(L, 4 + (1 if (pull and i in pushed) else 0))
            self._seg_args.append(L[-1][1])
            sync('tfx_fork', 2 * i + 1)
            grp = [(d, hd, dict(A=dy_a, lda=d, a_cols=d, B=self.og[i], ldb=hd, b_cols=hd, C=gp(f'{p}.1.fn.to_out.1.weight'), ldc=md.hd,
                                k_group=0 if md.dim_head == 64 else md.dim_head)),
                   (md.nqk, d, dict(algo_n=md.nq, A=dqkvg, lda=ldq, a_cols=ldq, B=self.ua[i], ldb=d, b_cols=d, C=gp(f'{p}.1.fn.to_qk.0.weight'), ldc=d,
                                    rowmap=ps._maps['heads'] if md.dim_head != 64 else None))]
            if md.has_skip(i):
                sk = self.xres[src[i]]
                grp.append((d, d, dict(A=G, lda=d, a_cols=d, B=x_in, ldb=d, b_cols=d, C=gp(f'{p}.0.weight'), ldc=2 * d)))
                grp.append((d, d, dict(A=G, lda=d, a_cols=d, B=sk, ldb=d, b_cols=d, C=gp(f'{p}.0.weight', d), ldc=2 * d)))
            self._tn_group(L, T, grp, side=side)
            per = -(-D // self.dp_groups) if self.dp_groups > 0 else D
            if I > 0 and i % per == 0:
                hi = min(i + per, D)
                off, cols = i * 2 * 3 * d, (hi - i) * 2 * 3 * d
                w_item = lambda it: L.append(Side(it) if side else it)
                w_item((lib.tfx_cast_block_bf16, (self.dtables.data_ptr() + 4 * off, nt3, self.dtab_bf.data_ptr() + 2 * off, nt3, I, cols)))
                self._tn(L, I, cols, 4 * d, side=side, A=self.dtab_bf.data_ptr() + 2 * off, lda=nt3, a_cols=cols, B=self.cond, ldb=4 * d, b_cols=4 * d,
                         C=gp(f'{p}.1.to_film.weight'), ldc=4 * d)
                w_item((lib.tfx_colsum_f32, (self.dtables.data_ptr() + 4 * off, nt3, I, cols, gp(f'{p}.1.to_film.bias'))))
            sync('tfx_join_record', i)
            if self.dp_groups > 0:
                if i % per == 0:
                    sync('tfx_join_wait', i)
                    self.bwd_cuts.append((len(L), i, min(i + per, D) - 1))
            if md.has_skip(i):
                st = S[f'skip_t{i}']
                self._nt(L, A=G, lda=d, B=st, ldb=d, M=T, N=d, K=d, epi=E['TFX_EPI_RESID'], C=self.gx[i], ldc=d, R=G, ldr=d)
                self._nt(L, A=G, lda=d, B=st[d:], ldb=d, M=T, N=d, K=d, epi=E['TFX_EPI_BF16'], C=self.dskip[src[i]], ldc=d)
                g = self.gx[i]
            else:
                g = G
        sync('tfx_join', 63)
        if pull:
            pull_launch(0, None, g, self.dx0, None)
            self._raw(L, lib.tfx_attnres_finish, self._src_tab.data_ptr(), D, d)
        else:
            self._raw(L, lib.tfx_add_bf16, g.data_ptr(), self.dH[0].data_ptr(), self.dx0.data_ptr(), T * d)
            if 0 in pushed:
                self._raw(L, lib.tfx_add_bf16, self.dx0.data_ptr(), self.dskip[0].data_ptr(), self.dx0.data_ptr(), T * d)
        self._raw(L, lib.tfx_onehot_bf16, self.text_ids.data_ptr(), self.tok_inst.data_ptr(), self.onehot.data_ptr(), T, md.vp)
        self._x0_param_grads(L, self.dx0)
        if I > 0:
            self._nt(L, A=self.dtab_bf, lda=nt3, B=S['ada_t'], ldb=nt3, M=I, N=4 * d, K=nt3, epi=E['TFX_EPI_BF16'], C=self.dcond, ldc=4 * d)
            self._raw(L, lib.tfx_silu_bwd, self.dcond.data_ptr(), self.pre.data_ptr(), self.dpre.data_ptr(), I * 4 * d)
            self._tn(L, I, 4 * d, d + 1, A=self.dpre, lda=4 * d, a_cols=4 * d, B=self.fe, ldb=md.kf, b_cols=md.kf,
                     C=gp('transformer.to_time_cond.1.weight'), ldc=d + 1)
            self._raw(L, lib.tfx_colsum_bf16, self.dpre.data_ptr(), 4 * d, I, 4 * d, None, None, gp('transformer.to_time_cond.1.bias'))

    def _x0_param_grads(self, L, dx0):
        md, T, d = self.md, self.T, self.md.dim
        gp, lib = self.ps.grad_ptr, capi.lib()
        self._tn(L, T, md.vocab, d, A=self.onehot, lda=md.vp, a_cols=md.vp, B=dx0, ldb=d, b_cols=d, C=gp('text_embed.weight'), ldc=d)
        for t, r in self.R.items():
            dl = md.dim_latents[t]; dlp = pad_to(dl, 64); lt = self.lat[t]
            if dl == d or t in self.ext:
                continue
            self._tn(L, r, d, dl, A=dx0, lda=d, a_cols=d, a_rowmap=self.row_gat[t], B=lt['xt'], ldb=dlp, b_cols=dlp,
                     C=gp(f'latent_to_model_projs.{t}.weight'), ldc=dl)
            cs = [dx0.data_ptr(), d, int(self.noise_args[t].R), d, None, self.row_tok[t].data_ptr(), gp(f'latent_to_model_projs.{t}.bias')]
            self._rows_dep[t].append((cs, 2))
            L.append((lib.tfx_colsum_bf16, cs))

    def set_taps(self, grads: dict, n_true: int):
        D, d = self.md.depth, self.md.dim
        self.clear_taps()
        if not grads:
            return
        if not self.pull:
            raise NotImplementedError('hidden taps need the pull-form AttentionResidual backward (depth <= 32 and dim <= 1024): the push form has no '
                                      'place where a hidden\'s gradient is formed once')
        for k, g in grads.items():
            assert 0 <= k <= D + 1
            buf = self.tap_buffer(k)
            if n_true < self.n:
                buf[:, n_true:].zero_()
            if g.data_ptr() != buf.data_ptr():
                buf[:, :n_true].copy_(g)
            if k == 0:
                lo = self.tap_buffer('0 lo')
                lo.zero_()
                if g.dtype != BF16:
                    lo[:, :n_true].copy_(g.float() - buf[:, :n_true].float())
                if self.tap0 is None:
                    self.tap0 = LaunchList()
                    for src in (buf, lo):
                        self._x0_param_grads(self.tap0, src)
            self.taps[k] = buf
            if 1 <= k <= D:
                self._pull_args[k].add = buf.data_ptr()

    def tap_buffer(self, k):
        buf = self._tap_buf.get(k)
        if buf is None:
            buf = self._tap_buf[k] = torch.zeros(self.b, self.n, self.md.dim, device=self.ps.device, dtype=BF16); self.nbytes += buf.numel() * 2
        return buf

    def clear_taps(self):
        for k in self.taps:
            if 1 <= k <= self.md.depth:
                self._pull_args[k].add = None
        self.taps = {}

    def run_bwd(self, stream, lo=0, hi=None):
        hi = len(self.bwd) if hi is None else hi
        taps = self.taps
        pos = self.tap_final
        if self.md.depth + 1 in taps and lo <= pos < hi:
            Plan.run(self.bwd, stream, lo, pos, graph='auto')
            dst, buf = self.dembed, taps[self.md.depth + 1]
            capi.check(capi.lib().tfx_add_bf16(dst.data_ptr(), buf.data_ptr(), dst.data_ptr(), dst.numel(), ctypes.c_void_p(stream)), 'tfx_add_bf16')
            lo = pos
        Plan.run(self.bwd, stream, lo, hi, graph='auto')
        if 0 in taps and hi == len(self.bwd):
            Plan.run(self.tap0, stream)

    def tap0_rows(self, index):
        if 0 not in self.taps:
            return None
        d = self.md.dim
        return self.taps[0].view(-1, d).index_select(0, index).float() + self.tap_buffer('0 lo').view(-1, d).index_select(0, index).float()

    @staticmethod
    def run(launches, stream, lo=0, hi=None, graph=False):
        lib = capi.lib()
        sp = ctypes.c_void_p(stream)
        if isinstance(launches, LaunchList):
            n = len(launches)
            lo = max(0, lo if lo >= 0 else n + lo)
            hi = n if hi is None else min(n, hi if hi >= 0 else n + hi)
            if hi <= lo:
# ... 27 lines not shown
```

transfusion_pytorch_amd/params.py:

```python
from __future__ import annotations

import math
from dataclasses import dataclass

import numpy as np
import torch
from torch import nn

from . import capi


def pad_to(x: int, m: int) -> int:
    return (x + m - 1) // m * m


@dataclass
class ModelDims:
    num_text_tokens: int
    dim: int
    depth: int
    heads: int
    dim_head: int
    dim_latents: tuple
    ff_expansion_factor: float = 4.
# ... 153 lines not shown
            for i in range(md.depth):
                at = order.index(f'transformer.layers.{i}.2.fn.net.3.bias') + 1
                order[at:at] = [f'transformer.layers.{i}.3.pseudo_queries', f'transformer.layers.{i}.3.norm_keys.gamma']
            assert sorted(order) == sorted(shapes)
            for name in order:
                shape = shapes[name]
                o = self.offsets[name][0]
                view = self.flat[o:o + int(np.prod(shape))].view(shape)
                if name.endswith('bias') and not name.endswith('to_ada_ln_zero.bias'):
                    view._fan_in_bound = 1. / math.sqrt(fan_in[name[:-len('bias')]])
                init_param_(name, view)
            for name in order:
                shape = shapes[name]
                o = self.offsets[name][0]
                view = self.flat[o:o + int(np.prod(shape))].view(shape)
                prm = nn.Parameter(view, requires_grad=True)
                self.params[name] = prm
                _attach(root, name, prm)
        _attach(root, 'transformer.to_time_cond.0.weights', self.fourier_w, buffer=True)
        self.rot_param = nn.Parameter(self.rot_freqs, requires_grad=False)
        _attach(root, 'rotary_emb.freqs', self.rot_param)
        self.shadows = {}
        self._shadow_version = None
        self._epoch = 0
        self._maps = {}
        self._jobs, self._job_table = [], None
        self._exp_ptrs = None
        self.device = torch.device('cpu')

    def view(self, name):
        o, shape = self.offsets[name]
        return self.flat[o:o + int(np.prod(shape))].view(shape)

    def grad_view(self, name):
        o, shape = self.offsets[name]
        return self.grad[o:o + int(np.prod(shape))].view(shape)

    def grad_ptr(self, name, elem_offset=0):
        return self.grad.data_ptr() + 4 * (self.offsets[name][0] + elem_offset)

    def ptr(self, name, elem_offset=0):
        return self.flat.data_ptr() + 4 * (self.offsets[name][0] + elem_offset)

    def reflatten(self, device):
        flat = torch.zeros(self.numel, device=device)
        with torch.no_grad():
            for name, shape in self.specs:
                o = self.offsets[name][0]
                v = flat[o:o + int(np.prod(shape))].view(shape)
                v.copy_(self.params[name].data)
                self.params[name].data = v
                self.params[name].grad = None
        self.flat = flat
        self.grad = torch.zeros(self.numel, device=device) if device.type == 'cuda' else None
        self.device = device
        self.shadows = {}
        self._shadow_version = None
        self._maps = {}

    def mark_dirty(self):
        self._shadow_version = None
        self._epoch += 1

    def params_version(self):
        ver = self.fourier_w._version + (self._epoch << 32)
        base = self.flat.data_ptr()
        exp = self._exp_ptrs
        if exp is None or exp[0] != base:
            exp = self._exp_ptrs = (base, [(name, prm, base + 4 * self.offsets[name][0]) for name, prm in self.params.items()])
        for name, prm, want in exp[1]:
            if prm.data_ptr() != want:
                v = self.view(name)
                if prm.shape != v.shape:
                    raise ValueError(f'parameter {name} was re-assigned with shape {tuple(prm.shape)}, the model was built for {tuple(v.shape)}')
                with torch.no_grad():
                    v.copy_(prm.data)
                prm.data = v
                self._shadow_version = None
            ver += prm._version
        return ver

    def ensure_grad_views(self):
        fresh = [n for n, p in self.params.items() if p.grad is None]
        if len(fresh) == len(self.params):
            self.grad.zero_()
        else:
            for n in fresh:
                self.grad_view(n).zero_()
        for n in fresh:
            self.params[n].grad = self.grad_view(n)

    def _map(self, key, arr):
        if key not in self._maps:
            self._maps[key] = torch.from_numpy(np.ascontiguousarray(arr, dtype=np.int32)).to(self.device)
        return self._maps[key]

    def _shadow(self, key, rows, cols):
        if key not in self.shadows:
            self.shadows[key] = torch.zeros(rows, cols, device=self.device, dtype=torch.bfloat16)
        return self.shadows[key]

    def _cast(self, stream, src_ptr, ld_src, Rs, Cs, dst, rowmap=None, transpose=False, n_rows_logical=None):
        ld_dst, Rd = dst.shape[1], dst.shape[0]
        assert ld_dst % 8 == 0
        nb = ((ld_dst + 63) // 64) * ((Rd + 63) // 64) if transpose else (Rd * ld_dst + 2047) // 2048
        self._jobs.append((dict(src=src_ptr, ld_src=ld_src, Rs=Rs, Cs=Cs, rowmap=capi.ptr(rowmap), dst=dst.data_ptr(), ld_dst=ld_dst, Rd=Rd,
                                Cd=n_rows_logical if transpose else ld_dst, transposed=int(transpose)), nb))

    def _launch_casts(self, stream):
        key = (self.flat.data_ptr(), len(self._jobs))
        if self._job_table is None or self._job_table[0] != key:
            J = capi.STRUCTS['tfx_cast_job']
            arr = (J * len(self._jobs))()
            first = 0
            for i, (f, nb) in enumerate(self._jobs):
                for k, v in f.items():
                    setattr(arr[i], k, v)
                arr[i].first_block = first
                first += nb
            import ctypes
            raw = torch.frombuffer(bytearray(ctypes.string_at(ctypes.addressof(arr), ctypes.sizeof(arr))), dtype=torch.uint8)
            self._job_table = (key, raw.to(self.device), len(self._jobs), first)
        _, tab, nj, nblk = self._job_table
        capi.check(capi.lib().tfx_cast_batch(tab.data_ptr(), nj, nblk, stream), 'tfx_cast_batch')

    def refresh_shadows(self, stream, force=False):
        ver = self.params_version()
        if not force and ver == self._shadow_version:
            return
        md = self.md
        d, hd, di, dip, D = md.dim, md.hd, md.di, md.dip, md.depth
        S, C = self._shadow, self._cast
        self._jobs = []
        C(stream, self.ptr('transformer.layers.0.1.to_film.weight'), 4 * d, md.nt3, 4 * d, S('ada', md.nt3, 4 * d))
        C(stream, self.ptr('transformer.layers.0.1.to_film.weight'), 4 * d, md.nt3, 4 * d, S('ada_t', 4 * d, md.nt3), transpose=True, n_rows_logical=md.nt3)
        C(stream, self.ptr('transformer.to_time_cond.1.weight'), d + 1, 4 * d, d + 1, S('time', 4 * d, md.kf))
        gmap = self._map('geglu', geglu_phys_to_ref_rows(di, dip))
        dh = md.dim_head
        if dh != 64:
            qmap = self._map('heads', head_phys_to_ref_rows(md.heads, dh))
            gam_map = self._map('gamma', np.where(np.arange(64) < dh, np.arange(64), -1))
        for i in range(D):
            p = f'transformer.layers.{i}'
            if md.has_skip(i):
                C(stream, self.ptr(f'{p}.0.weight'), 2 * d, d, 2 * d, S(f'skip{i}', d, 2 * d))
                C(stream, self.ptr(f'{p}.0.weight'), 2 * d, d, 2 * d, S(f'skip_t{i}', 2 * d, d), transpose=True, n_rows_logical=d)
            if dh == 64:
                C(stream, self.ptr(f'{p}.1.fn.to_qk.0.weight'), d, md.nq, d, S(f'qkvg{i}', md.nq, d))
                C(stream, self.ptr(f'{p}.1.fn.to_qk.0.weight'), d, md.nq, d, S(f'qkvg_t{i}', d, md.ldq), transpose=True, n_rows_logical=md.nq)
                C(stream, self.ptr(f'{p}.1.fn.to_out.1.weight'), hd, d, hd, S(f'out{i}', d, hd))
                C(stream, self.ptr(f'{p}.1.fn.to_out.1.weight'), hd, d, hd, S(f'out_t{i}', hd, d), transpose=True, n_rows_logical=d)
            else:
                hdk = md.hdk
                C(stream, self.ptr(f'{p}.1.fn.to_qk.0.weight'), d, md.nq, d, S(f'qkvg{i}', md.nqk, d), rowmap=qmap)
                C(stream, self.ptr(f'{p}.1.fn.to_qk.0.weight'), d, md.nq, d, S(f'qkvg_t{i}', d, md.ldq), rowmap=qmap, transpose=True, n_rows_logical=md.nqk)
                wo = self.ptr(f'{p}.1.fn.to_out.1.weight')
                C(stream, wo, dh, d * md.heads, dh, S(f'out{i}', d, hdk).view(d * md.heads, 64))
                ot = S(f'out_t{i}', hdk, d)
                for h in range(md.heads):
                    C(stream, wo + 4 * h * dh, hd, d, dh, ot[h * 64:(h + 1) * 64], transpose=True, n_rows_logical=d)
                for nm in ('q', 'k'):
                    key = f'g{nm}{i}'
                    if key not in self.shadows:
                        self.shadows[key] = torch.zeros(64, device=self.device)
                    capi.check(capi.lib().tfx_gather_f32(self.ptr(f'{p}.1.fn.{nm}_norm.gamma'), gam_map.data_ptr(), self.shadows[key].data_ptr(), 64, stream), 'gather_f32')
            C(stream, self.ptr(f'{p}.2.fn.net.0.weight'), d, 2 * di, d, S(f'ff1{i}', 2 * dip, d), rowmap=gmap)
            C(stream, self.ptr(f'{p}.2.fn.net.0.weight'), d, 2 * di, d, S(f'ff1_t{i}', d, 2 * dip), rowmap=gmap, transpose=True, n_rows_logical=2 * dip)
            C(stream, self.ptr(f'{p}.2.fn.net.3.weight'), di, d, di, S(f'ff2{i}', d, dip))
            C(stream, self.ptr(f'{p}.2.fn.net.3.weight'), di, d, di, S(f'ff2_t{i}', dip, d), transpose=True, n_rows_logical=d)
            b1 = self.shadows.get(f'ff1b{i}')
            if b1 is None:
                b1 = self.shadows[f'ff1b{i}'] = torch.zeros(2 * dip, device=self.device)
            capi.check(capi.lib().tfx_gather_f32(self.ptr(f'{p}.2.fn.net.0.bias'), gmap.data_ptr(), b1.data_ptr(), 2 * dip, stream), 'gather_f32')
# ... 16 lines not shown
```

transfusion_pytorch_amd/transfusion.py:

```python
from __future__ import annotations

import ctypes
import os
from typing import NamedTuple

import numpy as np
import torch
from torch import nn

from . import capi
from .engine import Plan
from .packing import fast_signature, is_int_tensor, scan_batch, scan_signature, token_maps, token_segments
from .axial import ContinuousAxialPositionalEmbedding
from .params import ModelDims, ParamStore


class LossBreakdown(NamedTuple):
    total: torch.Tensor
    text: torch.Tensor
    flow: list
    velocity: list | None = None
    recon: list | None = None


# ... 1361 lines not shown
            if dec is None:
                if self.modality_encoder[t] is not None:
                    raise ValueError('reconstruction loss with a modality encoder needs the matching modality decoder')
                lt['recw'].fill_(1. / rows)
                ra = plan._rec_args[t]
                ra.recon_mode, ra.grad_scale = 1, 2.0 * self.reconstruction_loss_weight / dl
                Plan.run(plan.rec, stream)
                recon_loss = plan.acc[2 + 2 * self.num_modalities + t] / dl
            else:
                with torch.no_grad():
                    tt = times.view(b, *([1] * (x.ndim - 1)))
                    rec = lt['eps'].view(x.shape) + lt['pred'].view(x.shape) * (1. - tt)
                    dec.eval()
                    recon_loss = torch.nn.functional.mse_loss(dec(rec.movedim(-1, 1) if self.channel_first_latent[t] else rec), orig_modalities.float())
            loss = loss + self.reconstruction_loss_weight * recon_loss
        self._step_id += 1
        self._live = (plan, self._step_id)
        emb_rows = None
        if torch.is_grad_enabled():
            if self._anchor is None or self._anchor.device != dev:
                self._anchor = torch.zeros((), device=dev, requires_grad=True)
            spec = {'in': [(k, ty) for k, ty, _ in rows_in], 'out': [t] if ext else []} if rows_in else _NO_ROWS
            loss, *emb_rows = _NativeLoss.apply(self._anchor, self, loss, spec, *[r for _, _, r in rows_in])
        elif ext:
            emb_rows = [plan.embed.float()]
        if ext:
            pred = self.model_to_latent_projs[t](emb_rows[0].view(b, *axial, d))
            if md.model_output_clean:
                pred = (pred - noised) / (1. - tt).clamp_min(md.clean_eps)
            flow_loss = torch.nn.functional.mse_loss(pred, flow_ext)
            loss = loss + flow_loss
            if self.has_recon_loss:
                rec = eps + pred * (1. - tt)
                if dec is not None:
                    with torch.no_grad():
                        dec.eval()
                        rec = dec(rec)
                recon_loss = torch.nn.functional.mse_loss(rec, orig_modalities.float())
                loss = loss + self.reconstruction_loss_weight * recon_loss
        if not return_loss_breakdown:
            return loss
        zero = torch.zeros((), device=dev)
        return loss, (flow_loss.detach(), velocity_loss.detach() if velocity_loss is not None else zero, recon_loss.detach() if recon_loss is not None else zero)

    @torch.no_grad()
    def generate_modality_only(self, batch_size=1, modality_type=None, fixed_modality_shape=None, modality_steps=16,
                               return_unprocessed_modalities=False):
        self._require_gpu()
        if self.num_modalities > 1 and modality_type is None:
            raise AssertionError('`modality_type` must be explicitly passed in on forward when training on greater than 1 modality')
        t = 0 if modality_type is None else int(modality_type)
        shape = fixed_modality_shape if fixed_modality_shape is not None else self.modality_default_shape[t]
        assert shape is not None
        dev = self.device
        y = self._gen_noise_override.to(dev, torch.float32).clone() if getattr(self, '_gen_noise_override', None) is not None \
            else torch.randn((batch_size, *shape, self.md.dim_latents[t]), device=dev)
        if self.channel_first_latent[t]:
            y = y.movedim(-1, 1).contiguous()
        was_training = self.training
        self.eval()
        try:
            grid = torch.linspace(0., 1., modality_steps, device=dev)
            f = lambda tt, yy: self.forward_modality(yy, times=tt.expand(batch_size), modality_type=t, encode_modality=False, return_loss=False)
            for i in range(modality_steps - 1):
                t0, dt = grid[i], grid[i + 1] - grid[i]
                y_mid = y + f(t0, y) * (dt * 0.5)
                y = y + dt * f(t0 + dt * 0.5, y_mid)
        finally:
            self.train(was_training)
        if self.modality_decoder[t] is not None:
            self.modality_decoder[t].eval()
            y = self.modality_decoder[t](y)
        return y

    def _native_backward(self, grad_out, step_id):
        plan, live_id = self._live
        if live_id != step_id:
            raise RuntimeError('backward() of a stale loss: the native engine keeps the activations of the latest forward only')
        if self._consumed == step_id:
            raise RuntimeError('backward() through the native Transfusion step a second time: the engine keeps one set of loss seeds per '
                               'forward (call forward again; retain_graph is not supported)')
        self._consumed = step_id
        ps = self.store
        ps.ensure_grad_views()
        go = grad_out.reshape(()).to(torch.float32)
        if self._bwd_scale is not None:
            go = go * self._bwd_scale
        lib, stream = capi.lib(), self._stream()
        sp = ctypes.c_void_p(stream)
        for seed in [plan.dlogits] + [lt['dpred'] for lt in plan.lat.values() if 'dpred' in lt]:
            capi.check(lib.tfx_scale_bf16_dev(seed.data_ptr(), seed.numel(), go.data_ptr(), sp), 'tfx_scale_bf16_dev')
        plan.dtables.zero_()
        if self.md.model_output_clean and plan.clean_mode == 'model' and len(plan.clean_bwd):
            Plan.run(plan.clean_bwd, stream)
        red = getattr(self, '_grad_reducer', None)
        if red is None or red.defer or not plan.bwd_cuts or not (torch.distributed.is_available() and torch.distributed.is_initialized()):
            if red is not None and red.defer:
                red.check_fresh()
            plan.run_bwd(stream)
            return
        red.check_fresh()
        red.begin()
        lo = 0
        for idx, first, last in plan.bwd_cuts:
            plan.run_bwd(stream, lo, idx)
            red.group_ready(first, last)
            lo = idx
        plan.run_bwd(stream, lo, None)

    @torch.no_grad()
    def sample_many(self, prompts=None, max_length=2048, text_temperature=1., text_min_p=0.1, fixed_modality_shape=None,
                    force_modality_at_start=None, init_modality_noise=None, modality_steps=16, return_unprocessed_modalities=False,
                    cfg_scale=3., _pos_emb_in_decode=False):
        from .sampling import Sampler
        was_training = self.training
        self.eval()
        try:
            if self._ext:
                plist = prompts if isinstance(prompts, list) else [prompts]
                outs = [self._sample_one_through_forward(pr, max_length=max_length, text_temperature=text_temperature, text_min_p=text_min_p, cache_kv=False,
                                                         fixed_modality_shape=fixed_modality_shape, force_modality_at_start=force_modality_at_start,
                                                         init_modality_noise=init_modality_noise, modality_steps=modality_steps, cfg_scale=cfg_scale)
                        for pr in plist]
                return outs if return_unprocessed_modalities else self.decode_modalities(outs)
            special = any(self.channel_first_latent) or any(e is not None for e in self.modality_encoder) or any(d is not None for d in self.modality_decoder)
            if special and prompts is not None:
                prompts = [self._normalize_prompt(pr) for pr in (prompts if isinstance(prompts, list) else [prompts])]
            out = Sampler(self).sample_many(prompts, max_length=max_length, text_temperature=text_temperature, text_min_p=text_min_p,
                                            fixed_modality_shape=fixed_modality_shape, force_modality_at_start=force_modality_at_start,
                                            init_modality_noise=init_modality_noise, modality_steps=modality_steps, cfg_scale=cfg_scale,
                                            pos_emb_in_decode=_pos_emb_in_decode)
            if special:
                out = [[(p[0], self._from_channel_last(p[0], p[1])) if isinstance(p, tuple) else p for p in sample] for sample in out]
                if not return_unprocessed_modalities:
                    out = self.decode_modalities(out)
            return out
        finally:
            self.train(was_training)

    def _normalize_prompt(self, pr):
        if pr is None:
            return None
        single = isinstance(pr, tuple) or torch.is_tensor(pr)
        parts = self._encode_modalities([[pr] if single else list(pr)])[0]
        out = []
        for part in parts:
            if torch.is_tensor(part) and part.is_floating_point():
                part = (0, part)
            if isinstance(part, tuple) and self.channel_first_latent[part[0]]:
                part = (part[0], part[1].movedim(0, -1))
            out.append(part)
        return out[0] if single else out

    @torch.no_grad()
    def sample_one(self, prompt=None, max_length=2048, text_temperature=1., text_min_p=0.1, cache_kv=None, fixed_modality_shape=None,
                   force_modality_at_start=None, init_modality_noise=None, modality_steps=16, return_unprocessed_modalities=False, cfg_scale=3.):
        if cache_kv is False and not self._ext and not self.model_output_clean:
            was_training = self.training
            self.eval()
            try:
                out = self._sample_one_through_forward(prompt, max_length=max_length, text_temperature=text_temperature, text_min_p=text_min_p, cache_kv=False,
                                                       fixed_modality_shape=fixed_modality_shape, force_modality_at_start=force_modality_at_start,
                                                       init_modality_noise=init_modality_noise, modality_steps=modality_steps, cfg_scale=cfg_scale)
                return out if return_unprocessed_modalities else self.decode_modalities(out)
            finally:
                self.train(was_training)
        return self.sample_many([prompt], max_length=max_length, text_temperature=text_temperature, text_min_p=text_min_p,
# ... 141 lines not shown
```

Before: 2541 samples/s.

## Fuse bias colsums into GEGLU-bwd and cast kernels; store weight grads when zero

The GEGLU backward GEMM epilogue now also accumulates the column sums used for the ff bias gradient, and the film-table cast kernel computes the to_film bias colsum in the same pass, so two separate colsum kernels go away. When all grads were freshly zeroed, weight-grad TN GEMMs with a single split and a destination no other product touches write plain stores, through a vectorized shared-memory staged path, instead of atomicAdds. An ABI version check is added so a stale library is rejected. The changes add atomics in the epilogue and tracking of which destinations are zero and do not overlap, which could be wrong if grads are accumulated across steps.

```diff
diff --git a/include/tfx.h b/include/tfx.h
--- a/include/tfx.h
+++ b/include/tfx.h
@@ -31,6 +31,7 @@
   float* qk_plan; float qk_softcap;
   tfx_bf16* qk_cache; int32_t qk_ld_cache; const int32_t* qk_cache_pos;
   const void* prefetch; int64_t prefetch_bytes;
+  float* colsum; const int32_t* colsum_map;
 } tfx_gemm_nt_args;
 int tfx_gemm_nt(const tfx_gemm_nt_args* a, void* stream);
 int tfx_gemm_nt_plan(const tfx_gemm_nt_args* a, int32_t* kind, int32_t* grid);
@@ -52,6 +53,7 @@
   float* colsum;
   int32_t k_group;
   const void* group_next;
+  int32_t c_is_zero;
 } tfx_gemm_tn_args;
 int tfx_gemm_tn(const tfx_gemm_tn_args* a, void* stream);
 int tfx_gemm_tn_plan(const tfx_gemm_tn_args* a, int32_t* kind, int32_t* tiles, int32_t* splits, int32_t* grid);
@@ -272,6 +274,7 @@
 int tfx_silu_bwd(const tfx_bf16* dy, const tfx_bf16* pre, tfx_bf16* dx, int64_t n, void* stream);
 int tfx_colsum_bf16(const tfx_bf16* src, int32_t ld, int32_t R, int32_t C, const int32_t* colmap, const int32_t* rowmap, float* out, void* stream);
 int tfx_colsum_f32(const float* src, int32_t ld, int32_t R, int32_t C, float* out, void* stream);
+int tfx_cast_colsum_block(const float* src, int32_t ld_src, tfx_bf16* dst, int32_t ld_dst, int32_t R, int32_t C, float* out, void* stream);
 int tfx_add_bf16(const tfx_bf16* a, const tfx_bf16* b, tfx_bf16* out, int64_t n, void* stream);
 int tfx_scale_bf16_dev(tfx_bf16* x, int64_t n, const float* scale, void* stream);
 int tfx_scale_bf16_copy(const tfx_bf16* src, tfx_bf16* dst, int64_t n, float scale, void* stream);
@@ -332,7 +335,7 @@
        TFX_OP_ADAM_STEP = 22, TFX_OP_DECODE_ATTN = 23, TFX_OP_LASER_V_FWD = 24, TFX_OP_LASER_V_BWD = 25, TFX_OP_COSINE_FWD_BWD = 26,
        TFX_OP_OUTPUT_TO_FLOW = 32, TFX_OP_GATHER_F32 = 33, TFX_OP_ONEHOT_BF16 = 34, TFX_OP_SCATTER_ROWS_BF16 = 35, TFX_OP_F32_TO_BF16 = 36,
        TFX_OP_SILU_BWD = 37, TFX_OP_COLSUM_BF16 = 38, TFX_OP_COLSUM_F32 = 39, TFX_OP_ADD_BF16 = 40, TFX_OP_SCALE_BF16_DEV = 41, TFX_OP_CAST_BLOCK_BF16 = 42, TFX_OP_SCALE_BF16_COPY = 43, TFX_OP_ADALN_POST_PRE_FWD = 44, TFX_OP_LAYER_END_FWD = 45,
-       TFX_OP_ATTNRES_PREP = 46, TFX_OP_ATTNRES_PULL_BWD = 47, TFX_OP_ATTNRES_FINISH = 52, TFX_OP_ADALN_PRE_POST_BWD = 53,
+       TFX_OP_ATTNRES_PREP = 46, TFX_OP_ATTNRES_PULL_BWD = 47, TFX_OP_ATTNRES_FINISH = 52, TFX_OP_ADALN_PRE_POST_BWD = 53, TFX_OP_CAST_COLSUM_BLOCK = 54,
        TFX_OP_FORK = 48, TFX_OP_JOIN = 49, TFX_OP_JOIN_RECORD = 50, TFX_OP_JOIN_WAIT = 51 };
 typedef struct { int32_t op; int32_t stream; const void* args; } tfx_launch;
 int tfx_run_list(const tfx_launch* list, int32_t n, void* stream, int32_t* failed_at);
@@ -344,6 +347,8 @@
 int tfx_set_single_stream(int32_t on);
 
 const char* tfx_version(void);
+enum { TFX_ABI = 7 };
+int tfx_abi(void);
 
 #ifdef __cplusplus
 }
diff --git a/transfusion_pytorch_amd/capi.py b/transfusion_pytorch_amd/capi.py
--- a/transfusion_pytorch_amd/capi.py
+++ b/transfusion_pytorch_amd/capi.py
@@ -82,6 +82,9 @@
             fn = getattr(L, fname)
             fn.restype = ret
             fn.argtypes = argt
+        if L.tfx_abi() != ENUMS['TFX_ABI']:
+            raise TfxError(f'{LIB_PATH} was built for ABI {L.tfx_abi()}, include/tfx.h is ABI {ENUMS["TFX_ABI"]}: rebuild it '
+                           '(`python -m transfusion_pytorch_amd.build --force`)')
         _lib = L
     return _lib
 
diff --git a/transfusion_pytorch_amd/csrc/gemm.hip b/transfusion_pytorch_amd/csrc/gemm.hip
--- a/transfusion_pytorch_amd/csrc/gemm.hip
+++ b/transfusion_pytorch_amd/csrc/gemm.hip
@@ -357,7 +357,7 @@
 #pragma unroll
     for (int q = 0; q < 2; q++) { const int m = m_w + i * 32 + q * 16 + (l >> 2); mo2[i][q] = (EPI == EPI_GEGLU && m < p.M) ? (p.rowmap ? p.rowmap[m] : m) : -1; }
   }
-  auto flush64 = [&](const bf16* s, int i, int n_base, int Nout) {
+  auto flush64 = [&](const bf16* s, int i, int n_base, int Nout, bool sum, float (&cs)[8]) {
     bf16x8 v[4];
 #pragma unroll
     for (int q = 0; q < 4; q++) {
@@ -367,7 +367,20 @@
 #pragma unroll
     for (int q = 0; q < 4; q++)
       if (n_base + ch * 8 < Nout && mo[i][q] >= 0) *(bf16x8*)((bf16*)p.C + (size_t)mo[i][q] * p.ldc + n_base + ch * 8) = v[q];
+    if (sum) {
+#pragma unroll
+      for (int q = 0; q < 4; q++)
+        if (n_base + ch * 8 < Nout && mo[i][q] >= 0) {
+#pragma unroll
+          for (int e = 0; e < 8; e++) cs[e] += bf2f(v[q][e]);
+        }
+    }
   };
+  float cs[2][8];
+#pragma unroll
+  for (int j = 0; j < 2; j++)
+#pragma unroll
+    for (int e = 0; e < 8; e++) cs[j][e] = 0.f;
   if constexpr (EPI == EPI_GEGLU) {
     f32x4 ba[4], bg[4];
     const f32x4 zero4 = {0.f, 0.f, 0.f, 0.f};
@@ -394,7 +407,7 @@
         }
         stage_put4(s, r, nl, u); stage_put4(s, r, 32 + nl, v); stage_put4_32(s + 2048, r, nl, h);
       }
-      flush64(s, i, n_w, p.N);
+      flush64(s, i, n_w, p.N, false, cs[0]);
       bf16x8 hv[2];
 #pragma unroll
       for (int q = 0; q < 2; q++) {
@@ -408,6 +421,7 @@
     }
   } else {
     bf16* sag = st + 2048;
+    const bool do_cs = p.colsum != nullptr;
     const int cbase = min(n_w >> 5, (p.N >> 5) - 2) * 64;
     bf16x8 pre[8];
     auto load_aux = [&](int i) {
@@ -442,7 +456,24 @@
           }
           stage_put4(st, r, 8 * g + 4 * hi, da); stage_put4(st, r, 32 + 8 * g + 4 * hi, dg);
         }
-        if (n_w + j * 32 < p.N) flush64(st, i, ((n_w >> 5) + j) * 64, 2 * p.N);
+        if (n_w + j * 32 < p.N) flush64(st, i, ((n_w >> 5) + j) * 64, 2 * p.N, do_cs, cs[j]);
+      }
+    }
+    if (do_cs) {
+#pragma unroll
+      for (int j = 0; j < 2; j++) {
+        float v = 0.f;
+#pragma unroll
+        for (int e = 0; e < 8; e++) {
+          float x = cs[j][e];
+          x += __shfl_xor(x, 8); x += __shfl_xor(x, 16); x += __shfl_xor(x, 32);
+          if ((l >> 3) == e) v = x;
+        }
+        const int col = ((n_w >> 5) + j) * 64 + ch * 8 + (l >> 3);
+        if (n_w + j * 32 < p.N && col < 2 * p.N) {
+          const int co = p.colsum_map ? p.colsum_map[col] : col;
+          if (co >= 0 && v != 0.f) atomicAdd(p.colsum + co, v);
+        }
       }
     }
   }
@@ -779,6 +810,9 @@
   return c < p.k_group ? (k >> 6) * p.k_group + c : -1;
 }
 
+TFX_DEV void tn_put(float* dst, float v, bool store) {
+  if (store) *dst = v; else atomicAdd(dst, v);
+}
 struct TnBlock { int tile, mbeg, mend; };
 TFX_DEV TnBlock tn_block(const GemmTN& p, int ntile) {
   const int per = gridDim.x >> 3;
@@ -899,7 +933,7 @@
         if (k < p.k_valid) {
           float v = acc[i][j][r] * p.alpha;
           const int ko = tn_out_col(p, k);
-          if (ko >= 0) atomicAdd(p.C + (size_t)no * p.ldc + ko, v);
+          if (ko >= 0) tn_put(p.C + (size_t)no * p.ldc + ko, v, p.c_is_zero != 0);
         }
       }
     }
@@ -1794,7 +1828,7 @@
       float* crow = p.C + (size_t)no * p.ldc;
 #pragma unroll
       for (int j = 0; j < FB; j++)
-        if (out_col[j] >= 0) atomicAdd(crow + out_col[j], acc[i][j][r] * p.alpha);
+        if (out_col[j] >= 0) tn_put(crow + out_col[j], acc[i][j][r] * p.alpha, p.c_is_zero != 0);
     }
   TN_STAMP(3)
 #ifdef TFX_TN_TIMING
@@ -1887,6 +1921,43 @@
         : OWT_CLOBBER);
   }
 
+  if (!SUM && p.c_is_zero) {
+    __syncthreads();
+    float* stg = (float*)smem_raw + w * (32 * 132);
+    const bool vec = p.k_group == 0 && (p.ldc & 3) == 0 && (((uintptr_t)p.C) & 15) == 0;
+    const int c4 = l & 31;
+    const int kc = k0 + wk * 128 + 4 * c4;
+#pragma unroll
+    for (int i = 0; i < 4; i++) {
+      int out_row[16];
+#pragma unroll
+      for (int q = 0; q < 16; q++) {
+        const int n = n0 + (wn * 4 + i) * 32 + 2 * q + hi;
+        out_row[q] = n >= p.N ? -1 : p.rowmap ? p.rowmap[n] : n;
+      }
+#pragma unroll
+      for (int j = 0; j < 4; j++)
+#pragma unroll
+        for (int r = 0; r < 16; r++) stg[((r & 3) + 8 * (r >> 2) + 4 * hi) * 132 + j * 32 + (l & 31)] = acc[i][j][r] * p.alpha;
+      asm volatile("" ::: "memory");
+#pragma unroll
+      for (int q = 0; q < 16; q++) {
+        const f32x4 v = *(const f32x4*)(stg + (2 * q + hi) * 132 + 4 * c4);
+        if (out_row[q] < 0) continue;
+        float* crow = p.C + (size_t)out_row[q] * p.ldc;
+        if (vec && kc + 3 < p.k_valid) *(f32x4*)(crow + kc) = v;
+        else {
+#pragma unroll
+          for (int e = 0; e < 4; e++) {
+            const int ko = kc + e < p.k_valid ? tn_out_col(p, kc + e) : -1;
+            if (ko >= 0) crow[ko] = v[e];
+          }
+        }
+      }
+      asm volatile("" ::: "memory");
+    }
+    return;
+  }
   int out_col[4];
 #pragma unroll
   for (int j = 0; j < 4; j++) {
@@ -2113,6 +2184,9 @@
   return tfx_qk_norm_rope_fwd(&a, (void*)s);
 }
 
+static bool geglu_bwd_stages(const GemmNT& p) {
+  return ((p.ldc | p.N) & 7) == 0 && (((uintptr_t)p.C) & 15) == 0 && (p.ldaux & 7) == 0 && (((uintptr_t)p.aux) & 15) == 0 && p.N >= 64;
+}
 int gemm_nt(const GemmNT& p, hipStream_t s) {
   if (p.K % BK != 0 || (p.A2 && p.K1 % BK != 0) || p.M <= 0 || p.N <= 0) return -1;
   if ((p.lda | p.ldb) & 7) return -2;
@@ -2122,7 +2196,14 @@
     case EPI_SILU: return launch_nt<EPI_SILU>(p, s);
     case EPI_RESID: return launch_nt<EPI_RESID>(p, s);
     case EPI_GEGLU: return (p.N % 64) ? -3 : launch_nt<EPI_GEGLU>(p, s);
-    case EPI_GEGLU_BWD: return (p.N % 64) ? -3 : launch_nt<EPI_GEGLU_BWD>(p, s);
+    case EPI_GEGLU_BWD: {
+      if (p.N % 64) return -3;
+      if (!p.colsum || (nt_plan(p).kind != NT_FALLBACK && geglu_bwd_stages(p))) return launch_nt<EPI_GEGLU_BWD>(p, s);
+      if (p.rowmap) return -6;
+      GemmNT q = p; q.colsum = nullptr;
+      const int rc = launch_nt<EPI_GEGLU_BWD>(q, s);
+      return rc ? rc : tfx_colsum_bf16((const tfx_bf16*)p.C, p.ldc, p.M, 2 * p.N, p.colsum_map, nullptr, p.colsum, (void*)s);
+    }
     case EPI_QKNR: return gemm_nt_qknr(p, s);
   }
   return -4;
@@ -2192,7 +2273,7 @@
   if (chunk < 192 || last < 192) return gp;
   gp.grid = (tiles * gp.splits + 7) / 8 * 8;
   if (head.splits == 0 && tiles * gp.splits < 0.8 * 256) return gp;
-  for (int i = 0; i < n; i++) gp.g.p[i].splits = gp.splits;
+  for (int i = 0; i < n; i++) { gp.g.p[i].splits = gp.splits; gp.g.p[i].c_is_zero = gp.g.p[i].c_is_zero && gp.splits == 1; }
   gp.ok = true;
   return gp;
 }
@@ -2222,10 +2303,11 @@
   if (p.M <= 0 || p.N <= 0 || p.K <= 0 || p.splits < 0) return -1;
   if ((p.lda | p.ldb | p.a_cols | p.b_cols) & 7) return -2;
   if (p.group_next) {
-    const TnGroupPlan gp = tn_group_plan(p);
+    TnGroupPlan gp = tn_group_plan(p);
     if (gp.ok) {
       bool sum = false;
       for (int i = 0; i < gp.count; i++) sum = sum || gp.g.p[i].colsum != nullptr;
+      if (sum) for (int i = 0; i < gp.count; i++) gp.g.p[i].c_is_zero = 0;
       const int ramp = tn_ramp(p.M, gp.tiles, gp.splits);
       static uint32_t attr_g0 = 0, attr_g1 = 0;
       if (sum) { ensure_smem_attr((const void*)gemm_tn_ow_group_kernel<true>, 131072, attr_g1); hipLaunchKernelGGL(gemm_tn_ow_group_kernel<true>, dim3(gp.grid), dim3(256), 131072, s, gp.g, ramp); }
@@ -2247,6 +2329,7 @@
   GemmTN q = p;
   const TnPlan pl = tn_plan(q);
   q.splits = pl.splits;
+  q.c_is_zero = p.c_is_zero && pl.splits == 1 && !(pl.kind == 3 && p.colsum);
   const int kind = pl.kind, grid = pl.grid;
   if (kind == 3) {
     static uint32_t attr_tnow = 0;
diff --git a/transfusion_pytorch_amd/csrc/runner.hip b/transfusion_pytorch_amd/csrc/runner.hip
--- a/transfusion_pytorch_amd/csrc/runner.hip
+++ b/transfusion_pytorch_amd/csrc/runner.hip
@@ -72,6 +72,8 @@
       return tfx_adaln_pre_post_bwd((const tfx_adaln_pre_args*)r->p0, (const tfx_adaln_post_args*)r->p1, s);
     case TFX_OP_CAST_BLOCK_BF16:
       return tfx_cast_block_bf16((const float*)r->p0, (int32_t)r->i0, (tfx_bf16*)r->p1, (int32_t)r->i1, (int32_t)r->i2, (int32_t)r->i3, s);
+    case TFX_OP_CAST_COLSUM_BLOCK:
+      return tfx_cast_colsum_block((const float*)r->p0, (int32_t)r->i0, (tfx_bf16*)r->p1, (int32_t)r->i1, (int32_t)r->i2, (int32_t)r->i3, (float*)r->p2, s);
     case TFX_OP_SCALE_BF16_COPY:
       return tfx_scale_bf16_copy((const tfx_bf16*)r->p0, (tfx_bf16*)r->p1, r->i0, r->f0, s);
     case TFX_OP_SCALE_BF16_DEV:
diff --git a/transfusion_pytorch_amd/csrc/tokenwise.hip b/transfusion_pytorch_amd/csrc/tokenwise.hip
--- a/transfusion_pytorch_amd/csrc/tokenwise.hip
+++ b/transfusion_pytorch_amd/csrc/tokenwise.hip
@@ -1868,6 +1868,49 @@
   }
 }
 
+__global__ __launch_bounds__(256) void cast_colsum_block_k(const float* src, int ld_src, bf16* dst, int ld_dst, int R, int C, float* out, int rows_per_block) {
+  __shared__ float s[4][64][9];
+  const int cx = threadIdx.x & 63, ry = threadIdx.x >> 6;
+  const int c0 = (blockIdx.x * 64 + cx) * 8;
+  const int rbeg = blockIdx.y * rows_per_block, rend = min(R, rbeg + rows_per_block);
+  float a[8];
+#pragma unroll
+  for (int e = 0; e < 8; e++) a[e] = 0.f;
+  if (c0 < C) {
+    auto put = [&](int r, const f32x4& lo, const f32x4& hi) {
+      bf16x8 o;
+#pragma unroll
+      for (int e = 0; e < 4; e++) { o[e] = f2bf(lo[e]); o[4 + e] = f2bf(hi[e]); a[e] += lo[e]; a[4 + e] += hi[e]; }
+      *(bf16x8*)(dst + (size_t)r * ld_dst + c0) = o;
+    };
+    int r = rbeg + ry;
+    for (; r + 12 < rend; r += 16) {
+      f32x4 lo[4], hi[4];
+#pragma unroll
+      for (int u = 0; u < 4; u++) { const float* q = src + (size_t)(r + 4 * u) * ld_src + c0; lo[u] = *(const f32x4*)q; hi[u] = *(const f32x4*)(q + 4); }
+#pragma unroll
+      for (int u = 0; u < 4; u++) put(r + 4 * u, lo[u], hi[u]);
+    }
+    for (; r < rend; r += 4) {
+      const float* q = src + (size_t)r * ld_src + c0;
+      const f32x4 lo = *(const f32x4*)q, hi = *(const f32x4*)(q + 4);
+      put(r, lo, hi);
+    }
+  }
+#pragma unroll
+  for (int e = 0; e < 8; e++) s[ry][cx][e] = a[e];
+  __syncthreads();
+#pragma unroll
+  for (int k = 0; k < 2; k++) {
+    const int idx = threadIdx.x + 256 * k, cc = idx >> 3, e = idx & 7;
+    const int col = (blockIdx.x * 64 + cc) * 8 + e;
+    if (col < C) {
+      const float v = ((s[0][cc][e] + s[1][cc][e]) + s[2][cc][e]) + s[3][cc][e];
+      if (v != 0.f) atomicAdd(out + col, v);
+    }
+  }
+}
+
 __global__ __launch_bounds__(256) void sumsq_k(const float* g, long long n, float* out) {
   __shared__ float sacc[WAVES];
   float s = 0.f;
@@ -2209,6 +2252,13 @@
   int rpb = colsum_rows_per_block(R);
   hipLaunchKernelGGL(colsum_k<float>, dim3((C + 63) / 64, (R + rpb - 1) / rpb), dim3(256), 0, ST(s), src, ld, R, C, (const int*)nullptr, (const int*)nullptr, out, rpb); RET();
 }
+int tfx_cast_colsum_block(const float* src, int32_t ld_src, tfx_bf16* dst, int32_t ld_dst, int32_t R, int32_t C, float* out, void* s) {
+  if (R <= 0 || C <= 0) return 0;
+  if (!src || !dst || !out) return -1;
+  if ((C | ld_src | ld_dst) & 7 || (((uintptr_t)src | (uintptr_t)dst) & 15)) return -2;
+  int rpb = (R + 63) / 64; if (rpb < 16) rpb = 16;
+  hipLaunchKernelGGL(cast_colsum_block_k, dim3((C + 511) / 512, (R + rpb - 1) / rpb), dim3(256), 0, ST(s), src, ld_src, (bf16*)dst, ld_dst, R, C, out, rpb); RET();
+}
 int tfx_sumsq(const float* g, int64_t n, float* out, void* s) {
   if (n == 0) return 0;
   long long blocks = (n / 4 + 255) / 256; if (blocks > 2048) blocks = 2048; if (blocks < 1) blocks = 1;
@@ -2260,6 +2310,7 @@
   if (nch >= (1ll << 31)) return -4;
   hipLaunchKernelGGL(laser_v_bwd_k, dim3((unsigned)((nch + 255) / 256)), dim3(256), 0, ST(s), *a, (unsigned)nch); RET();
 }
-const char* tfx_version(void) { return "tfx-hip gfx950 r4-laser-muon-selfflow"; }
-
-}
+const char* tfx_version(void) { return "tfx-hip gfx950 r4-laser-muon-selfflow abi7"; }
+int tfx_abi(void) { return TFX_ABI; }
+
+}
diff --git a/transfusion_pytorch_amd/engine.py b/transfusion_pytorch_amd/engine.py
--- a/transfusion_pytorch_amd/engine.py
+++ b/transfusion_pytorch_amd/engine.py
@@ -31,6 +31,44 @@
     return src
 
 
+
+
+def tn_products(lists):
+    lib = capi.lib()
+
+    def plan(a):
+        out = [ctypes.c_int32(-9) for _ in range(4)]
+        capi.check(lib.tfx_gemm_tn_plan(ctypes.byref(a), *[ctypes.byref(o) for o in out]), 'tfx_gemm_tn_plan')
+        return tuple(o.value for o in out)
+
+    res = []
+    for lst in lists:
+        for fn, a in lst:
+            if fn != 'tfx_gemm_tn':
+                continue
+            chain = [a] + list(getattr(a, '_chain', []))
+            if len(chain) > 1:
+                kind, tiles, splits, _ = plan(a)
+                if kind == 3 and tiles == sum(-(-m.N // 256) * -(-m.K // 256) for m in chain):
+                    res += [(m, splits) for m in chain]
+                    continue
+            for m in chain:
+                one = type(m).from_buffer_copy(m)
+                one.group_next = None
+                res.append((m, plan(one)[2]))
+    return res
+
+
+def zero_dest_products(lists):
+    prods = tn_products(lists)
+    span = lambda a: (int(a.C), int(a.C) + 4 * ((a.N - 1) * a.ldc + a.k_valid))
+    spans = [span(a) for a, _ in prods]
+    out = []
+    for k, (a, splits) in enumerate(prods):
+        lo, hi = spans[k]
+        if splits == 1 and not any(j != k and lo2 < hi and lo < hi2 for j, (lo2, hi2) in enumerate(spans)):
+            out.append(a)
+    return out
 
 
 _LAUNCH = capi.STRUCTS['tfx_launch']
@@ -727,11 +765,11 @@
                         first=1 if i == D - 1 else 0, dgamma=gp(f'{p}.3.norm_keys.gamma'), dpq=gp(f'{p}.3.pseudo_queries'))
                 L.append(('tfx_adaln_post_bwd', a_postf))
             self._nt(L, algo_n=di, A=dy_f, lda=d, B=S[f'ff2_t{i}'], ldb=d, M=T, N=dip, K=d, epi=E['TFX_EPI_GEGLU_BWD'], C=dag, ldc=2 * dip,
-                     aux=self.ag[i], ldaux=2 * dip)
+                     aux=self.ag[i], ldaux=2 * dip, colsum=gp(f'{p}.2.fn.net.0.bias'), colsum_map=gmap)
             sync('tfx_fork', 2 * i)
             ff_grp = [(d, di, dict(A=dy_f, lda=d, a_cols=d, B=self.hm[i], ldb=dip, b_cols=dip, C=gp(f'{p}.2.fn.net.3.weight'), ldc=di)),
                       (2 * dip, d, dict(algo_n=2 * di, A=dag, lda=2 * dip, a_cols=2 * dip, B=self.uf[i], ldb=d, b_cols=d, rowmap=gmap,
-                                        C=gp(f'{p}.2.fn.net.0.weight'), ldc=d, colsum=gp(f'{p}.2.fn.net.0.bias')))]
+                                        C=gp(f'{p}.2.fn.net.0.weight'), ldc=d))]
             self._tn_group(L, T, ff_grp, side=side)
             self._nt(L, algo_k=2 * di, A=dag, lda=2 * dip, B=S[f'ff1_t{i}'], ldb=2 * dip, M=T, N=d, K=2 * dip, epi=E['TFX_EPI_BF16'], C=self.du, ldc=d)
             a_pref = capi.make_args('tfx_adaln_pre_args', T=T, d=d, x=self.xb[i], tok_inst=self.tok_inst, table=tf, ld_table=nt3,
@@ -787,10 +825,10 @@
                 hi = min(i + per, D)
                 off, cols = i * 2 * 3 * d, (hi - i) * 2 * 3 * d
                 w_item = lambda it: L.append(Side(it) if side else it)
-                w_item((lib.tfx_cast_block_bf16, (self.dtables.data_ptr() + 4 * off, nt3, self.dtab_bf.data_ptr() + 2 * off, nt3, I, cols)))
+                w_item((lib.tfx_cast_colsum_block, (self.dtables.data_ptr() + 4 * off, nt3, self.dtab_bf.data_ptr() + 2 * off, nt3, I, cols,
+                                                    gp(f'{p}.1.to_film.bias'))))
                 self._tn(L, I, cols, 4 * d, side=side, A=self.dtab_bf.data_ptr() + 2 * off, lda=nt3, a_cols=cols, B=self.cond, ldb=4 * d, b_cols=4 * d,
                          C=gp(f'{p}.1.to_film.weight'), ldc=4 * d)
-                w_item((lib.tfx_colsum_f32, (self.dtables.data_ptr() + 4 * off, nt3, I, cols, gp(f'{p}.1.to_film.bias'))))
             sync('tfx_join_record', i)
             if self.dp_groups > 0:
                 if i % per == 0:
@@ -819,6 +857,12 @@
             self._tn(L, I, 4 * d, d + 1, A=self.dpre, lda=4 * d, a_cols=4 * d, B=self.fe, ldb=md.kf, b_cols=md.kf,
                      C=gp('transformer.to_time_cond.1.weight'), ldc=d + 1)
             self._raw(L, lib.tfx_colsum_bf16, self.dpre.data_ptr(), 4 * d, I, 4 * d, None, None, gp('transformer.to_time_cond.1.bias'))
+
+        self._zero_tn = zero_dest_products([self.clean_bwd, self.bwd])
+
+    def set_grads_zero(self, fresh: bool):
+        for a in self._zero_tn:
+            a.c_is_zero = 1 if fresh else 0
 
     def _x0_param_grads(self, L, dx0):
         md, T, d = self.md, self.T, self.md.dim
diff --git a/transfusion_pytorch_amd/params.py b/transfusion_pytorch_amd/params.py
--- a/transfusion_pytorch_amd/params.py
+++ b/transfusion_pytorch_amd/params.py
@@ -259,13 +259,15 @@
 
     def ensure_grad_views(self):
         fresh = [n for n, p in self.params.items() if p.grad is None]
-        if len(fresh) == len(self.params):
+        all_fresh = len(fresh) == len(self.params)
+        if all_fresh:
             self.grad.zero_()
         else:
             for n in fresh:
                 self.grad_view(n).zero_()
         for n in fresh:
             self.params[n].grad = self.grad_view(n)
+        return all_fresh
 
     def _map(self, key, arr):
         if key not in self._maps:
diff --git a/transfusion_pytorch_amd/transfusion.py b/transfusion_pytorch_amd/transfusion.py
--- a/transfusion_pytorch_amd/transfusion.py
+++ b/transfusion_pytorch_amd/transfusion.py
@@ -1467,7 +1467,7 @@
                                'forward (call forward again; retain_graph is not supported)')
         self._consumed = step_id
         ps = self.store
-        ps.ensure_grad_views()
+        plan.set_grads_zero(ps.ensure_grad_views())
         go = grad_out.reshape(()).to(torch.float32)
         if self._bwd_scale is not None:
             go = go * self._bwd_scale
```

Result: no change. 2553 samples/s (median of 6 runs) (+0.5%).
